# muonzoo/cutesdr

Hardware: AMD Instinct MI355X
Metric: complex IQ MSamples/s through CFastFIR+demod chain; achieved HBM GB/s vs peak (higher is better)
Workload: dtype f32; 1 GPU; C3: 256 channels/GPU x 2^19 IQ samples, 16384-pt CFastFIR overlap-save (8193 taps, hop 8192), shared -5..+5 kHz filter @62.5 kS/s; channels_per_gpu=256, samples_per_channel=524288, fft_size=16384, parallelism=channels sharded x1, no data-path collective

## Files before the change

cutesdr_amd/csrc/capi_fastfir.hip:

```cpp
#include "capi_common.hpp"
#include "capi_internal.hpp"
#include <algorithm>
#include "fastfir_kernels.h"
#include "fastfir_design_kernels.h"
#include "host_math.hpp"
#include "patch_queue.hpp"
#include <cmath>
#include <cstdlib>
#include <cstring>
#include <vector>

using namespace csdr;

static int log2_of(int n)
{
    int l = 0;
    while ((1 << l) < n) l++;
    return ((1 << l) == n) ? l : -1;
}

struct csdr_fastfir_batch {
    int device, channels, n, log2n;
    int cus;
    hipStream_t last_stream;
    bool per_channel;
    float *d_h;
    float *d_h2;
    float *d_hist;
    int hist_cur;
    int dbg_stage; float *dbg_out;
    int variant;
    float *d_tw1, *d_tw2;
    double flo, fhi, off, fs;
    std::vector<std::vector<cd>> resp;
    std::vector<int> perm, perm2;
    PatchQueue patches;
    std::vector<DesignJob> jobs;
    std::vector<int> job_of;
    std::vector<char> stale;
    double *d_win = nullptr, *d_tw = nullptr;
    int *d_perm = nullptr, *d_perm2 = nullptr;
    double *d_resp = nullptr;
    hipEvent_t ev_design = nullptr;
};

static void cancel_job(csdr_fastfir_batch *b, int slot)
{
    const int i = b->job_of[slot];
    if (i < 0) return;
    b->job_of[slot] = -1;
    if ((size_t)i + 1 != b->jobs.size()) { b->jobs[i] = b->jobs.back(); b->job_of[b->jobs[i].slot] = i; }
    b->jobs.pop_back();
}

static void queue_job(csdr_fastfir_batch *b, int slot, double nfc, double nfs)
{
    const DesignJob j{slot, 0, nfc, nfs};
    if (b->job_of[slot] >= 0) b->jobs[b->job_of[slot]] = j;
    else { b->job_of[slot] = (int)b->jobs.size(); b->jobs.push_back(j); }
    b->stale[slot] = 1;
}

static int flush_control(csdr_fastfir_batch *b, hipStream_t s)
{
    if (b->jobs.empty()) return b->patches.flush(s);
    unsigned char *h = nullptr, *d = nullptr;
    int rc = b->patches.take(b->jobs.size() * sizeof(DesignJob), &h, &d);
    if (rc) return rc;
    memcpy(h, b->jobs.data(), b->jobs.size() * sizeof(DesignJob));
    rc = b->patches.launch(s);
    hipError_t e = hipSuccess;
    if (!rc) {
        DesignArgs a;
        a.jobs = (const DesignJob *)d; a.win = b->d_win; a.tw = b->d_tw; a.perm = b->d_perm; a.perm2 = b->d_perm2;
        a.h = b->d_h; a.h2 = b->d_h2; a.resp = b->d_resp;
        e = fastfir_design_launch(b->log2n, a, (int)b->jobs.size(), s);
        if (e == hipSuccess) {
            for (const DesignJob &j : b->jobs) b->job_of[j.slot] = -1;
            b->jobs.clear();
            if (!b->ev_design) e = hipEventCreateWithFlags(&b->ev_design, hipEventDisableTiming);
            if (e == hipSuccess) e = hipEventRecord(b->ev_design, s);
        }
    }
    const int rr = b->patches.retire(s);
    if (rc) return rc;
    if (e != hipSuccess) return fail(CSDR_EHIP, "filter design launch: %s", hipGetErrorString(e));
    return rr;
}

static int fetch_mirror(csdr_fastfir_batch *b, int slot)
{
    if (!b->stale[slot]) return CSDR_OK;
    const int rc = flush_control(b, b->last_stream);
    if (rc) return rc;
    if (b->ev_design) CSDR_HIP(hipEventSynchronize(b->ev_design));
    CSDR_HIP(hipMemcpy(b->resp[slot].data(), b->d_resp + (size_t)slot * 2 * b->n, sizeof(cd) * (size_t)b->n, hipMemcpyDeviceToHost));
    b->stale[slot] = 0;
    return CSDR_OK;
}

static int design_state(csdr_fastfir_batch *b)
{
    if (b->d_resp) return CSDR_OK;
    const size_t n = (size_t)b->n, p = n / 2 + 1;
    const auto win = fastfir_window((int)p);
    const auto tw = design_twiddles(n);
    if (!b->d_win) CSDR_HIP(hipMalloc((void **)&b->d_win, p * sizeof(double)));
    if (!b->d_tw) CSDR_HIP(hipMalloc((void **)&b->d_tw, n * sizeof(double)));
    if (!b->d_perm) CSDR_HIP(hipMalloc((void **)&b->d_perm, n * sizeof(int)));
    if (!b->d_perm2) CSDR_HIP(hipMalloc((void **)&b->d_perm2, n * sizeof(int)));
    CSDR_HIP(hipMemcpy(b->d_win, win->data(), p * sizeof(double), hipMemcpyHostToDevice));
    CSDR_HIP(hipMemcpy(b->d_tw, tw.data(), n * sizeof(double), hipMemcpyHostToDevice));
    CSDR_HIP(hipMemcpy(b->d_perm, b->perm.data(), n * sizeof(int), hipMemcpyHostToDevice));
    CSDR_HIP(hipMemcpy(b->d_perm2, b->perm2.data(), n * sizeof(int), hipMemcpyHostToDevice));
    CSDR_HIP(hipMalloc((void **)&b->d_resp, (size_t)b->channels * n * sizeof(cd)));
    return CSDR_OK;
}

static void build_perm(csdr_fastfir_batch *b)
{
    const int T = b->n / 32;
    b->perm.resize(b->n);
    for (int j = 0; j < 16; j++)
        for (int t = 0; t < T; t++)
            for (int e = 0; e < 2; e++)
                b->perm[(j * T + t) * 2 + e] = fastfir_bin_of(b->log2n, t, 2 * j + e);
    b->perm2.clear();
    {
        b->perm2.resize(b->n);
        for (int j = 0; j < 16; j++)
            for (int t = 0; t < T; t++)
                for (int e = 0; e < 2; e++) b->perm2[(j * T + t) * 2 + e] = fastfir2_bin_of(b->log2n, t, j, e);
    }
}

static int upload_response(csdr_fastfir_batch *b, int slot, const std::vector<cd> &H)
{
    std::vector<float> dev(2 * (size_t)b->n);
    for (int pass = 0; pass < 2; pass++) {
        const std::vector<int> &perm = pass ? b->perm2 : b->perm;
        float *dst = pass ? b->d_h2 : b->d_h;
        if (perm.empty() || !dst) continue;
        for (int i = 0; i < b->n; i++) {
            const cd v = H[perm[i]];
            dev[2 * i] = (float)v.real();
            dev[2 * i + 1] = (float)v.imag();
        }
        const int rc = b->patches.add(dst + (size_t)slot * 2 * b->n, dev.data(), dev.size() * sizeof(float));
        if (rc) return rc;
    }
    return CSDR_OK;
}

static int set_response(csdr_fastfir_batch *b, int slot, const std::vector<cd> &H)
{
    cancel_job(b, slot);
    const int rc = upload_response(b, slot, H);
    if (rc) return rc;
    b->resp[slot] = H;
    b->stale[slot] = 0;
    return CSDR_OK;
}

extern "C" {

csdr_fastfir_batch *csdr_fastfir_batch_create(int device, int channels, int fft_size)
{
    const int l2 = log2_of(fft_size);
    if (l2 < 11 || l2 > 14 || channels < 1) {
        fail(CSDR_EINVAL, "fft_size must be 2048..16384 (power of two), channels >= 1");
        return nullptr;
    }
    if (!device_ok(device)) return nullptr;
    csdr_fastfir_batch *b = new csdr_fastfir_batch();
    b->device = device; b->channels = channels; b->n = fft_size; b->log2n = l2;
    b->per_channel = false; b->hist_cur = 0; b->dbg_stage = 0; b->dbg_out = nullptr;
    b->last_stream = nullptr;
    {
        int cus = 0;
        if (hipDeviceGetAttribute(&cus, hipDeviceAttributeMultiprocessorCount, device) != hipSuccess || cus <= 0) cus = 256;
        b->cus = cus;
    }
    {
        const char *v = getenv("CSDR_FASTFIR_VARIANT");
        b->variant = (v && atoi(v) == 0) ? 0 : 2;
    }
    b->d_h = b->d_h2 = b->d_hist = b->d_tw1 = b->d_tw2 = nullptr;
    b->flo = -1.0; b->fhi = 1.0; b->off = 1.0; b->fs = 1.0;
    build_perm(b);
    const size_t hbytes = (size_t)fft_size * 8, histbytes = 2 * (size_t)channels * (fft_size / 2) * 8;
    std::vector<float> tw1(2 * 1024), tw2(2 * 1024);
    for (int i = 0; i < 1024; i++) {
        const double a = kTwoPi * (double)i / (double)fft_size;
        tw1[2 * i] = (float)std::cos(a); tw1[2 * i + 1] = (float)std::sin(a);
    }
    for (int k = 0; k < 32; k++)
        for (int i = 0; i < 32; i++) {
            const double a = kTwoPi * (double)(i * k) / 1024.0;
            tw2[2 * (k * 32 + i)] = (float)std::cos(a); tw2[2 * (k * 32 + i) + 1] = (float)std::sin(a);
        }
    bool ok = hipMalloc((void **)&b->d_h, hbytes) == hipSuccess &&
              hipMalloc((void **)&b->d_h2, hbytes) == hipSuccess && hipMemset(b->d_h2, 0, hbytes) == hipSuccess &&
              hipMalloc((void **)&b->d_hist, histbytes) == hipSuccess &&
              hipMalloc((void **)&b->d_tw1, 8192) == hipSuccess &&
              hipMalloc((void **)&b->d_tw2, 8192) == hipSuccess &&
              hipMemset(b->d_h, 0, hbytes) == hipSuccess &&
              hipMemset(b->d_hist, 0, histbytes) == hipSuccess &&
              hipMemcpy(b->d_tw1, tw1.data(), 8192, hipMemcpyHostToDevice) == hipSuccess &&
              hipMemcpy(b->d_tw2, tw2.data(), 8192, hipMemcpyHostToDevice) == hipSuccess;
    if (!ok) {
        fail(CSDR_ENOMEM, "device allocation failed: %s", hipGetErrorString(hipGetLastError()));
        csdr_fastfir_batch_destroy(b);
        return nullptr;
    }
    b->resp.assign(1, std::vector<cd>(fft_size, cd(0, 0)));
    b->job_of.assign(channels, -1);
    b->stale.assign(channels, 0);
    return b;
}

void csdr_fastfir_batch_destroy(csdr_fastfir_batch *b)
{
    if (!b) return;
    (void)hipSetDevice(b->device);
    if (b->d_h) (void)hipFree(b->d_h);
    if (b->d_h2) (void)hipFree(b->d_h2);
    if (b->d_hist) (void)hipFree(b->d_hist);
    if (b->d_tw1) (void)hipFree(b->d_tw1);
    if (b->d_tw2) (void)hipFree(b->d_tw2);
    if (b->ev_design) { (void)hipEventSynchronize(b->ev_design); (void)hipEventDestroy(b->ev_design); }
    if (b->d_win) (void)hipFree(b->d_win);
    if (b->d_tw) (void)hipFree(b->d_tw);
    if (b->d_perm) (void)hipFree(b->d_perm);
    if (b->d_perm2) (void)hipFree(b->d_perm2);
    if (b->d_resp) (void)hipFree(b->d_resp);
    delete b;
}

int csdr_fastfir_batch_setup(csdr_fastfir_batch *b, int channel, double flo, double fhi,
                             double offset, double fs)
{
    if (!b || channel < -1 || channel >= b->channels) return fail(CSDR_EINVAL, "bad handle/channel");
    if (!device_ok(b->device)) return CSDR_EHIP;
    if (channel < 0) {
        if (!b->per_channel && flo == b->flo && fhi == b->fhi && offset == b->off && fs == b->fs) return 0;
        b->flo = flo; b->fhi = fhi; b->off = offset; b->fs = fs;
    }
    std::vector<cd> H;
    if (!fastfir_design(b->n, flo, fhi, offset, fs, H))
        return fail(CSDR_EINVAL, "filter parameter error (reference keeps the previous taps)");
    if (channel >= 0 && !b->per_channel) {
        { const int rcm = fetch_mirror(b, 0); if (rcm) return rcm; }
        { const int rcp = flush_control(b, b->last_stream); if (rcp) return rcp; }
        CSDR_HIP(hipDeviceSynchronize());
        float *nh = nullptr;
        const size_t one = (size_t)b->n * 8;
        CSDR_HIP(hipMalloc((void **)&nh, one * b->channels));
        for (int c = 0; c < b->channels; c++)
            CSDR_HIP(hipMemcpy((char *)nh + one * c, b->d_h, one, hipMemcpyDeviceToDevice));
        CSDR_HIP(hipFree(b->d_h));
        b->d_h = nh;
        if (b->d_h2) {
            float *nh2 = nullptr;
            CSDR_HIP(hipMalloc((void **)&nh2, one * b->channels));
            for (int c = 0; c < b->channels; c++)
                CSDR_HIP(hipMemcpy((char *)nh2 + one * c, b->d_h2, one, hipMemcpyDeviceToDevice));
            CSDR_HIP(hipFree(b->d_h2));
            b->d_h2 = nh2;
        }
        b->resp.resize(b->channels, b->resp[0]);
        b->per_channel = true;
    }
    if (channel < 0 && b->per_channel) {
        for (int c = 0; c < b->channels; c++) {
            int rc = set_response(b, c, H);
            if (rc) return rc;
        }
    } else {
        int rc = set_response(b, channel < 0 ? 0 : channel, H);
        if (rc) return rc;
    }
    return 1;
}

int csdr_fastfir_batch_setup_many(csdr_fastfir_batch *b, int n, const int *channel, const double *flo, const double *fhi,
                                  const double *offset, const double *fs, int *status)
{
    if (!have_device()) return CSDR_EHIP;
    if (!b || n < 0 || (n > 0 && (!channel || !flo || !fhi || !offset || !fs || !status)))
        return fail(CSDR_EINVAL, "bad handle, negative count or null array");
    for (int i = 0; i < n; i++)
        if (channel[i] < -1 || channel[i] >= b->channels) return fail(CSDR_EINVAL, "entry %d: channel %d", i, channel[i]);
    if (n == 0) return CSDR_OK;
    if (!device_ok(b->device)) return CSDR_EHIP;
    { const int rc = design_state(b); if (rc) return rc; }
    for (int i = 0; i < n; i++) {
        const int ch = channel[i];
        if (ch < 0) {
            if (!b->per_channel && flo[i] == b->flo && fhi[i] == b->fhi && offset[i] == b->off && fs[i] == b->fs) { status[i] = 0; continue; }
            b->flo = flo[i]; b->fhi = fhi[i]; b->off = offset[i]; b->fs = fs[i];
        }
        double nfc, nfs;
        if (!fastfir_design_job(flo[i], fhi[i], offset[i], fs[i], nfc, nfs)) { status[i] = CSDR_EINVAL; continue; }
        if (ch >= 0 && !b->per_channel) {
            const int rc = csdr_fastfir_batch_setup(b, ch, flo[i], fhi[i], offset[i], fs[i]);
            if (rc < 0) { for (int j = i; j < n; j++) status[j] = rc; return rc; }
        }
        if (ch < 0 && b->per_channel) for (int c = 0; c < b->channels; c++) queue_job(b, c, nfc, nfs);
        else queue_job(b, ch < 0 ? 0 : ch, nfc, nfs);
        status[i] = 1;
    }
    return CSDR_OK;
}

int csdr_fastfir_batch_reset(csdr_fastfir_batch *b)
{
    if (!b) return fail(CSDR_EINVAL, "bad handle");
    if (!device_ok(b->device)) return CSDR_EHIP;
    CSDR_HIP(hipMemset(b->d_hist, 0, 2 * (size_t)b->channels * (b->n / 2) * 8));
    return CSDR_OK;
}

int csdr_fastfir_batch_get_response(csdr_fastfir_batch *b, int channel, double *h_out)
{
    if (!b || !h_out || channel < 0 || channel >= b->channels) return fail(CSDR_EINVAL, "bad argument");
    const int slot = b->per_channel ? channel : 0;
    if (b->stale[slot]) {
        if (!device_ok(b->device)) return CSDR_EHIP;
        const int rc = fetch_mirror(b, slot);
        if (rc) return rc;
    }
    const std::vector<cd> &H = b->resp[slot];
    memcpy(h_out, H.data(), sizeof(cd) * H.size());
    return CSDR_OK;
}

int csdr_fastfir_batch_process(csdr_fastfir_batch *b, const float *d_in, long long in_stride,
                               int n_per_channel, float *d_out, long long out_stride,
                               void *stream, int blocks_per_wg)
{
    if (!b || !d_in || !d_out) return fail(CSDR_EINVAL, "bad handle or null buffer");
    const int L = b->n / 2;
    if (n_per_channel <= 0 || n_per_channel % L != 0)
        return fail(CSDR_EINVAL, "n_per_channel (%d) must be a positive multiple of the hop %d", n_per_channel, L);
    if (in_stride < n_per_channel || out_stride < n_per_channel)
        return fail(CSDR_EINVAL, "channel stride shorter than n_per_channel");
    if (((uintptr_t)d_in | (uintptr_t)d_out) & 15 || (in_stride & 1) || (out_stride & 1))
        return fail(CSDR_EINVAL, "buffers must be 16-byte aligned and strides even");
    if ((long long)n_per_channel * 8 >= (1ll << 31))
        return fail(CSDR_EINVAL, "n_per_channel (%d) too large for one call: at most %d samples", n_per_channel, (1 << 28) - L);
    if (!device_ok(b->device)) return CSDR_EHIP;
    hipStream_t s = (hipStream_t)stream;
    b->last_stream = s;
    { const int rcp = flush_control(b, s); if (rcp) return rcp; }
    FastFirArgs a;
    const size_t hist_half = (size_t)b->channels * L * 2;
    a.in = (const v2f_h *)d_in; a.out = (v2f_h *)d_out;
    a.hist = (const v2f_h *)(b->d_hist + b->hist_cur * hist_half);
    a.hist_next = (v2f_h *)(b->d_hist + (b->hist_cur ^ 1) * hist_half);
    a.h = (const v4f_h *)b->d_h; a.tw1 = (const v2f_h *)b->d_tw1; a.tw2 = (const v2f_h *)b->d_tw2;
    a.in_stride = in_stride; a.out_stride = out_stride;
    a.h_stride = b->per_channel ? b->n / 2 : 0;
    a.channels = b->channels;
    a.nblocks = n_per_channel / L;
    if (blocks_per_wg <= 0) {
        const long per_cu = b->n >= 16384 ? 1 : (b->n >= 8192 ? 2 : (b->n >= 4096 ? 4 : 8));
        const long slots = (long)b->cus * per_cu;
        long best_runs = 1; double best_eff = -1.0;
        const long max_runs = std::min<long>(a.nblocks, std::max<long>(1, 4 * ((slots + b->channels - 1) / b->channels)));
        for (long runs = 1; runs <= max_runs; runs++) {
            const long wgs = runs * b->channels;
            const double eff = (double)wgs / (double)(((wgs + slots - 1) / slots) * slots);
            if (eff > best_eff + 1e-9) { best_eff = eff; best_runs = runs; }
        }
        blocks_per_wg = (int)((a.nblocks + best_runs - 1) / best_runs);
    }
    if (blocks_per_wg > a.nblocks) blocks_per_wg = a.nblocks;
    a.blocks_per_run = blocks_per_wg;
    a.runs = (a.nblocks + blocks_per_wg - 1) / blocks_per_wg;
    a.dbg_stage = b->dbg_stage; a.dbg = (v2f_h *)b->dbg_out;
    if (b->variant >= 2) {
        a.h = (const v4f_h *)b->d_h2;
        CSDR_HIP(fastfir2_launch(b->log2n, a, s));
    }
    else CSDR_HIP(fastfir_launch(b->log2n, a, s));
    b->hist_cur ^= 1;
    return CSDR_OK;
}

int csdr__fastfir_batch_copy_row(csdr_fastfir_batch *dst, int dr, csdr_fastfir_batch *src, int sr)
{
    if (!dst || !src || dst->n != src->n || dr < 0 || dr >= dst->channels || sr < 0 || sr >= src->channels)
        return fail(CSDR_EINVAL, "bad argument");
    if (!device_ok(dst->device)) return CSDR_EHIP;
    CSDR_HIP(hipDeviceSynchronize());
    const int L = dst->n / 2;
    const size_t shalf = (size_t)src->channels * L * 2, dhalf = (size_t)dst->channels * L * 2;
    CSDR_HIP(hipMemcpy(dst->d_hist + dst->hist_cur * dhalf + (size_t)dr * L * 2,
                       src->d_hist + src->hist_cur * shalf + (size_t)sr * L * 2, (size_t)L * 8, hipMemcpyDeviceToDevice));
    const int sslot = src->per_channel ? sr : 0;
    { const int rcm = fetch_mirror(src, sslot); if (rcm) return rcm; }
    const std::vector<cd> &H = src->resp[sslot];
    if (dst->channels > 1 && !dst->per_channel) return fail(CSDR_ESTATE, "destination rows share one filter");
    const int slot = dst->per_channel ? dr : 0;
    int rc = set_response(dst, slot, H);
    if (rc) return rc;
    dst->flo = dst->fhi = dst->off = dst->fs = std::nan("");
    return CSDR_OK;
}

int csdr__fastfir_set_variant(csdr_fastfir_batch *b, int variant)
{
    if (!b || (variant != 0 && variant != 2)) return CSDR_EINVAL;
    b->variant = variant;
    return CSDR_OK;
}

int csdr__dbg_fastfir_stage(csdr_fastfir_batch *b, int stage, float *d_dbg)
{
    if (!b) return CSDR_EINVAL;
    b->dbg_stage = stage; b->dbg_out = d_dbg;
    return CSDR_OK;
}

}

struct csdr_fastfir {
    csdr_fastfir_batch *b;
    int n, pending;
    PinnedBuf pin_in, pin_out;
    hipStream_t s = nullptr;
    float *d_in, *d_out;
    size_t cap;
};

static int ensure_cap(csdr_fastfir *f, size_t samples)
{
    if (samples <= f->cap) return CSDR_OK;
    if (f->d_in) (void)hipFree(f->d_in);
    if (f->d_out) (void)hipFree(f->d_out);
    f->d_in = f->d_out = nullptr; f->cap = 0;
    CSDR_HIP(hipMalloc((void **)&f->d_in, samples * 8));
    CSDR_HIP(hipMalloc((void **)&f->d_out, samples * 8));
    f->cap = samples;
    return CSDR_OK;
}

extern "C" {

csdr_fastfir *csdr_fastfir_create(int device, int fft_size)
{
    csdr_fastfir_batch *b = csdr_fastfir_batch_create(device, 1, fft_size);
    if (!b) return nullptr;
    csdr_fastfir *f = new csdr_fastfir();
    f->b = b; f->n = fft_size; f->pending = 0; f->d_in = f->d_out = nullptr; f->cap = 0;
    if (hipStreamCreateWithFlags(&f->s, hipStreamNonBlocking) != hipSuccess) { csdr_fastfir_destroy(f); fail(CSDR_EHIP, "stream creation failed"); return nullptr; }
    return f;
}

void csdr_fastfir_destroy(csdr_fastfir *f)
{
    if (!f) return;
    (void)hipSetDevice(f->b->device);
    if (f->d_in) (void)hipFree(f->d_in);
    if (f->d_out) (void)hipFree(f->d_out);
    if (f->s) { (void)hipStreamSynchronize(f->s); (void)hipStreamDestroy(f->s); }
    csdr_fastfir_batch_destroy(f->b);
    delete f;
}

int csdr_fastfir_setup(csdr_fastfir *f, double flo, double fhi, double offset, double fs)
{
    if (!f) return fail(CSDR_EINVAL, "bad handle");
    return csdr_fastfir_batch_setup(f->b, -1, flo, fhi, offset, fs);
}

int csdr_fastfir_process(csdr_fastfir *f, int n, const double *in_iq, double *out_iq)
{
    if (!f || n < 0 || (n > 0 && (!in_iq || !out_iq))) return fail(CSDR_EINVAL, "bad argument");
    if (n == 0) return 0;
    if (!device_ok(f->b->device)) return CSDR_EHIP;
    const int L = f->n / 2;
    int rc = f->pin_in.reserve(2 * ((size_t)f->pending + n));
    if (rc) return rc;
    cvt_to_f32(f->pin_in.p + 2 * (size_t)f->pending, in_iq, 2 * (size_t)n);
    const int avail = f->pending + n;
    const int nproc = (avail / L) * L;
    if (nproc == 0) { f->pending = avail; return 0; }
    if ((rc = ensure_cap(f, (size_t)nproc))) { f->pending = avail; return rc; }
    if ((rc = f->pin_out.reserve(2 * (size_t)nproc))) { f->pending = avail; return rc; }
    CSDR_HIP(hipMemcpyAsync(f->d_in, f->pin_in.p, (size_t)nproc * 8, hipMemcpyHostToDevice, f->s));
    rc = csdr_fastfir_batch_process(f->b, f->d_in, nproc, nproc, f->d_out, nproc, (void *)f->s, 0);
    if (rc) {
        (void)hipStreamSynchronize(f->s);
        f->pending = avail;
        return rc;
    }
    CSDR_HIP(hipMemcpyAsync(f->pin_out.p, f->d_out, (size_t)nproc * 8, hipMemcpyDeviceToHost, f->s));
    CSDR_HIP(hipStreamSynchronize(f->s));
    cvt_to_f64(out_iq, f->pin_out.p, 2 * (size_t)nproc);
    f->pending = avail - nproc;
    if (f->pending > 0) memmove(f->pin_in.p, f->pin_in.p + 2 * (size_t)nproc, 2 * (size_t)f->pending * sizeof(float));
    return nproc;
}

}
```

cutesdr_amd/csrc/capi_hosttest.hip:

```cpp
#include "capi_common.hpp"
#include "host_math.hpp"
#include "dc_host.hpp"
#include "pc_host.hpp"
#include "display_plan.hpp"
#include "testgen_host.hpp"
#include "scope_host.hpp"
#include "fastfir_kernels.h"
#include <cstring>

using namespace csdr;

extern "C" {

int csdr__host_fastfir_design(int n, double flo, double fhi, double off, double fs, double *h_out)
{
    std::vector<cd> H;
    if (!fastfir_design(n, flo, fhi, off, fs, H)) return -1;
    memcpy(h_out, H.data(), sizeof(cd) * n);
    return 0;
}
int csdr__host_design_job(double flo, double fhi, double off, double fs, double *nfc, double *nfs)
{
    return fastfir_design_job(flo, fhi, off, fs, *nfc, *nfs) ? 0 : -1;
}
int csdr__host_fastfir_bin_of(int log2n, int t, int r) { return fastfir_bin_of(log2n, t, r); }

int csdr__host_dc_plan(double in_rate, double bw, int *codes, double *out_rate, int *warmup)
{
    DcPlan p = dc_make_plan(in_rate, bw);
    for (int i = 0; i < p.nstages; i++) codes[i] = p.kind[i];
    *out_rate = p.out_rate; *warmup = p.W;
    return p.nstages;
}
int csdr__host_dc_stage_taps(double in_rate, double bw, int s, double *h)
{
    DcPlan p = dc_make_plan(in_rate, bw);
    if (s < 0 || s >= p.nstages) return -1;
    const DcStage &st = p.st[s];
    const int L = st.hist + (p.kind[s] == 3 ? 2 : 1);
    for (int i = 0; i < L; i++) h[i] = 0;
    if (st.center >= 0) h[st.center] = st.ccoef;
    for (int q = 0; q < st.npairs; q++) { h[st.a[q]] = st.c[q]; h[st.b[q]] = st.c[q]; }
    return L;
}
void csdr__host_dc_nco(double freq, double cw, double in_rate, unsigned long long *inc, double *stored)
{
    DcHostChan c;
    c.in_rate = in_rate; c.cw_offset = cw;
    c.set_frequency(freq);
    *inc = c.inc; *stored = c.nco_freq;
}
int csdr__host_fir_design(int kind, double scale, double astop, double fpass, double fstop, double fs,
                          double hilbert_off, double *coef, double *icoef, double *qcoef)
{
    HostFir f;
    if (kind == 0) f.init_lp(scale, astop, fpass, fstop, fs);
    else f.init_hp(scale, astop, fpass, fstop, fs);
    if (hilbert_off != 0.0) f.gen_hilbert(hilbert_off);
    for (int i = 0; i < f.ntaps; i++) { coef[i] = f.coef[i]; icoef[i] = f.icoef[i]; qcoef[i] = f.qcoef[i]; }
    return f.ntaps;
}
void csdr__host_iir_design(int kind, double f0, double q, double fs, double *c5)
{
    PcIir f;
    iir_design(f, kind, f0, q, fs);
    c5[0] = f.b0; c5[1] = f.b1; c5[2] = f.b2; c5[3] = f.a1; c5[4] = f.a2;
}
void csdr__host_agc_params(int on, int hang, int thresh, int manual, int slope, int decay, double fs, double *out12)
{
    HostAgc h;
    PcAgc d;
    memset(&d, 0, sizeof(d));
    h.set(d, on != 0, hang != 0, thresh, manual, slope, decay, fs);
    out12[0] = d.knee; out12[1] = d.gain_slope; out12[2] = d.fixed_gain; out12[3] = d.manual_gain;
    out12[4] = d.att_rise; out12[5] = d.att_fall; out12[6] = d.dec_rise; out12[7] = d.dec_fall;
    out12[8] = d.dly_n; out12[9] = d.win_n; out12[10] = d.hang_time; out12[11] = 0;
}

void csdr__host_display_plan(const int *state5, long long n, int N, long long *out8)
{
    DisplayState s;
    s.pos = state5[0]; s.skip = state5[1]; s.counter = state5[2]; s.gated = state5[3]; s.ready = state5[4];
    const DisplayPlan p = display_plan(s, n, N);
    out8[0] = p.start; out8[1] = p.step; out8[2] = p.count;
    out8[3] = p.next.pos; out8[4] = p.next.skip; out8[5] = p.next.counter; out8[6] = p.next.gated; out8[7] = p.next.ready;
}
int csdr__host_display_skip_value(double sample_rate, int fft_size, int max_display_rate)
{
    return display_skip_value(sample_rate, fft_size, max_display_rate);
}

unsigned long long csdr__host_tg_first_crossing(double x0, double d, double limit, int strict, double *value)
{
    return tg::first_crossing(x0, d, limit, strict != 0, value);
}
double csdr__host_tg_value_at(double x0, double d, unsigned long long index) { return tg::value_at(x0, d, index); }
void csdr__host_tg_pulse_pattern(double fs, double period, double width, unsigned long long *K, unsigned long long *W)
{
    tg::Gen g;
    g.fs = fs; g.period = period; g.width = width;
    g.pulse_pattern();
    *K = g.K; *W = g.W;
}
void *csdr__host_tg_create(void) { tg::Gen *g = new tg::Gen(); g->reset(); g->on = true; return g; }
void csdr__host_tg_destroy(void *h) { delete (tg::Gen *)h; }
void csdr__host_tg_slot(void *h, int what, double v)
{
    tg::Gen &g = *(tg::Gen *)h;
    switch (what) {
    case 0: g.on_sweep_start(v); break;
    case 1: g.on_sweep_stop(v); break;
    case 2: g.on_sweep_rate(v); break;
    case 3: g.on_pulse_width(v); break;
    case 4: g.on_pulse_period(v); break;
    case 5: g.on_signal_pwr(v); break;
    case 6: g.on_noise_pwr(v); break;
    default: g.reset(); break;
    }
}
int csdr__host_tg_run(void *h, int n, double fs, unsigned long long *phase, int *gate)
{
    tg::Gen &g = *(tg::Gen *)h;
    if (g.fs != fs) { g.fs = fs; g.pulse_valid = false; g.reset(); }
    tg::ChanParam p;
    g.pulse((uint32_t)n, p);
    uint32_t done = 0;
    int launches = 0;
    while (done < (uint32_t)n) {
        p.nseg = 0;
        const uint32_t lo = done;
        done += g.advance(done, (uint32_t)n - done, p);
        launches++;
        for (uint32_t j = lo; j < done; j++) {
            uint32_t s = 0;
            for (uint32_t k = 1; k < p.nseg; k++) s += p.seg_start[k] <= j;
            const uint64_t t = j - p.seg_start[s];
            const tg::u128 P = (((tg::u128)p.seg_p[s][1] << 64) | p.seg_p[s][0])
                + (((tg::u128)p.seg_d[s][1] << 64) | p.seg_d[s][0]) * (tg::u128)t
                + (((tg::u128)p.seg_d2[s][1] << 64) | p.seg_d2[s][0]) * (tg::u128)(t * (t - 1) / 2);
            phase[j] = (uint64_t)(P >> 64);
            const uint64_t m = (uint64_t)j + 1;
            const uint64_t pos = m < p.wrap1 ? p.pos0 + m : (m - p.wrap1) % p.period;
            gate[j] = !p.gate_on || pos < p.width;
        }
    }
    return launches;
}

long long csdr__host_scope_emissions(long long inpos, int pos, double pix, double sr, int w, long long n, long long max_out,
                                     long long *samples, long long *end3)
{
    const sc::Plan p = sc::make_plan(inpos, pos, pix, sr, w, n);
    for (long long e = 0; e < p.emits && e < max_out; e++) samples[e] = p.sample(e);
    end3[0] = p.emits; end3[1] = p.pos_end; end3[2] = p.inpos_end;
    return p.emits;
}
void csdr__host_scope_settings(int span_ms, int display_rate, double sr, int w, double *pix, int *skip)
{
    *pix = sc::pixel_time(span_ms, w); *skip = sc::skip_value(span_ms, display_rate, sr);
}
void csdr__host_scope_free_run(long long cnt, int skip, long long m, long long *out3)
{
    const sc::FreeRun r = sc::free_run(cnt, skip, m);
    out3[0] = r.displays; out3[1] = r.last; out3[2] = r.cnt;
}
struct HostScope {
    sc::Chan ch;
    sc::ChanState st;
    int w = 100, h = 100;
    int ring[2 * sc::kMaxW], screen[2 * sc::kMaxW];
};
void *csdr__host_scope_create(void)
{
    HostScope *s = new HostScope();
    memset(&s->st, 0, sizeof(s->st)); s->st.skipcounter = -2;
    memset(s->ring, 0, sizeof(s->ring)); memset(s->screen, 0, sizeof(s->screen));
    s->ch.derive(s->w);
    return s;
}
void csdr__host_scope_destroy(void *h) { delete (HostScope *)h; }
void csdr__host_scope_slot(void *h, int what, int v, int v2)
{
    HostScope &s = *(HostScope *)h;
    switch (what) {
    case 0: s.w = v; s.h = v2; s.ch.reset(v); break;
    case 1: s.ch.on_horz_span(v, s.w); break;
    case 2: s.ch.on_display_rate(v); break;
    case 3: s.ch.on_trigger_mode(v, s.w); break;
    case 4: s.ch.level = v; break;
    case 5: s.ch.vert = v; break;
    case 6: s.ch.reset(s.w); break;
    default: s.ch.time_plot_done(); break;
    }
}
long long csdr__host_scope_put(void *h, const float *re, const float *im, int n, double fs)
{
    HostScope &s = *(HostScope *)h;
    sc::ChanParam par;
    s.ch.prepare(n, fs, s.w, par);
    sc::ChanState &st = s.st;
    int *ring = s.ring, *screen = s.screen;
    const int w = s.w;
    if (par.flags & sc::F_RESET) memset(ring, 0, sizeof(s.ring));
    sc::apply_flags(st, par.flags);
    if (par.n > 0) {
        const sc::Plan pl = sc::make_plan(st.inpos, st.pos, par.pix, par.sr, w, par.n);
        const long long E = pl.emits;
        const int pos0 = st.pos;
        auto get = [&](long long e, int &a, int &b) { const long long k = pl.sample(e); a = sc::sat_int(re[k]); b = im ? sc::sat_int(im[k]) : 0; };
        long long trig = -1;
        if (sc::searches(st, par))
            for (long long e = 0; e < E && trig < 0; e++) {
                int cur, prv, t;
                get(e, cur, t);
                if (e == 0) prv = st.prev; else get(e - 1, prv, t);
                if (sc::crossing(par.mode, par.level, cur, prv)) trig = e;
            }
        const sc::Display d = sc::decide(st, par, w, E, trig);
        if (d.at >= 0)
            for (int i = 0; i < w; i++) {
                int a, b, slot = 0;
                const long long e = sc::screen_source(d, i, w, pos0, &slot);
                if (e >= 0) get(e, a, b); else { a = ring[slot]; b = ring[sc::kMaxW + slot]; }
                screen[i] = a; screen[sc::kMaxW + i] = b;
            }
        for (long long e = E > w ? E - w : 0; e < E; e++) {
            int a, b;
            get(e, a, b);
            const int slot = (int)((pos0 + e) % w);
            ring[slot] = a; ring[sc::kMaxW + slot] = b;
        }
        int t;
        if (E > 0) get(E - 1, st.prev, t);
        st.inpos = pl.inpos_end; st.pos = pl.pos_end;
    }
    return st.emits;
}
void csdr__host_scope_get(void *h, long long *state7, int *screen_re, int *screen_im)
{
    HostScope &s = *(HostScope *)h;
    const sc::ChanState &st = s.st;
    state7[0] = st.inpos; state7[1] = st.pos; state7[2] = st.prev; state7[3] = st.trigstate; state7[4] = st.trigcounter;
    state7[5] = st.trigbufpos; state7[6] = st.skipcounter;
    memcpy(screen_re, s.screen, sizeof(int) * s.w); memcpy(screen_im, s.screen + sc::kMaxW, sizeof(int) * s.w);
}
int csdr__host_scope_sat_int(double x) { return sc::sat_int(x); }

}
```

cutesdr_amd/csrc/fastfir2_kernels.hip:

```cpp
#define CSDR_FMA_BFLY 1
#define CSDR_PLAIN_CONST_FMA 1
#include "launch_once.hpp"
#include "fastfir_dev.hpp"
#include "fastfir_kernels.h"

namespace csdr {

#define CSDR_SB() __builtin_amdgcn_sched_barrier(0)

#ifndef K1_LDAUX
#define K1_LDAUX 2
#endif
#ifndef K1_STAUX
#define K1_STAUX 2
#endif
#ifndef K1_HREG
#define K1_HREG 8
#endif
#ifndef K1_HREG4K
#define K1_HREG4K 4
#endif
#ifndef K1_W1_FETCH_MAX_R0
#define K1_W1_FETCH_MAX_R0 2
#endif
#ifndef K1_HREG2K
#define K1_HREG2K 8
#endif

#ifdef CSDR_K1_STAMPS
#define CSDR_STAMP(i)                                                                         \
    do {                                                                                      \
        CSDR_SB();                                                                            \
        unsigned long long now_;                                                              \
        asm volatile("s_memtime %0\n\ts_waitcnt lgkmcnt(0)" : "=s"(now_)::"memory");         \
        CSDR_SB();                                                                            \
        acc_[i] += now_ - last_;                                                              \
        last_ = now_;                                                                         \
    } while (0)
#else
#define CSDR_STAMP(i) do { } while (0)
#endif

#define CSDR_PRIO(p) __builtin_amdgcn_s_setprio(p)

#ifdef K1_ABLATE
__device__ __forceinline__ void keep_alive(v4f v) { asm volatile("" ::"v"(v)); }
#endif

template <int LOG2N>
struct K1Cfg {
    using Base = FastFirCfg<LOG2N>;
    static constexpr int VW = LOG2N == 12 ? 2 : (LOG2N == 11 ? 4 : 1);
    static constexpr int TV = Base::T;
    static constexpr int T = VW * TV;
    static constexpr int LDS_BYTES = (VW * Base::LDS_DATA + 1024) * 8;
};

template <int LOG2N>
__global__ __launch_bounds__(K1Cfg<LOG2N>::T) __attribute__((amdgpu_waves_per_eu(2, 2)))
void fastfir_os2_kernel(FastFirArgs a)
{
    CSDR_WG_TRACE_SCOPE(a.trace, WGT_FF);
    using Cfg = FastFirCfg<LOG2N>;
    constexpr int N = Cfg::N, T = Cfg::T, R0 = Cfg::R0, G = Cfg::G, L = N / 2;
    constexpr int HALF = R0 / 2;
    constexpr int VW = K1Cfg<LOG2N>::VW;
    constexpr int HREG = LOG2N == 12 ? K1_HREG4K : (LOG2N == 11 ? K1_HREG2K : K1_HREG);
    static_assert(R0 == 16 || R0 == 8 || R0 == 4 || R0 == 2, "the grouped outer pass is written for N = 2048 ... 16384");
    auto block_barrier = [] {
        if constexpr (LOG2N == 11) {
            __builtin_amdgcn_fence(__ATOMIC_RELEASE, "wavefront"); __builtin_amdgcn_wave_barrier(); __builtin_amdgcn_fence(__ATOMIC_ACQUIRE, "wavefront");
        } else {
            __syncthreads();
        }
    };
    extern __shared__ __attribute__((aligned(16))) unsigned char smem_raw[];
    const int t = VW == 1 ? (int)threadIdx.x : (int)threadIdx.x % T, vw = VW == 1 ? 0 : (int)threadIdx.x / T;
    v2f *lds = reinterpret_cast<v2f *>(smem_raw) + vw * Cfg::LDS_DATA;
    v2f *tw2 = reinterpret_cast<v2f *>(smem_raw) + VW * Cfg::LDS_DATA;
    if constexpr (VW > 1) {
        for (int i = threadIdx.x; i < 1024; i += VW * T) tw2[i] = a.tw2[i];
        __syncthreads();
    }

    int wg = blockIdx.x * VW + vw, ch, run;
    if ((a.channels & 7) == 0) {
        int xcd = wg & 7, slot = wg >> 3;
        ch = (slot / a.runs) * 8 + xcd;
        run = slot % a.runs;
    } else {
        ch = wg / a.runs;
        run = wg % a.runs;
    }
    const int b0 = run * a.blocks_per_run;
    int b1 = b0 + a.blocks_per_run;
    if (b1 > a.nblocks) b1 = a.nblocks;
#if defined(__HIP_DEVICE_COMPILE__) && !defined(__gfx950__)
#error "fastfir_os2_kernel<12> relies on gfx950's s_barrier ignoring terminated waves (two virtual workgroups per workgroup)"
#endif
    if (ch >= a.channels || b0 >= b1) return;

    if constexpr (VW == 1)
        for (int i = t; i < 1024; i += T) tw2[i] = a.tw2[i];

    const rsrc_t r_in = make_rsrc(a.in + (long)ch * a.in_stride, (unsigned)a.nblocks * L * 8u);
    const rsrc_t r_hist = make_rsrc(a.hist + (long)ch * L, L * 8u);
    const rsrc_t r_out = make_rsrc(a.out + (long)ch * a.out_stride, (unsigned)a.nblocks * L * 8u);
    const rsrc_t r_h = make_rsrc(a.h + (long)ch * a.h_stride, N * 8u);
    constexpr int PSTEP = 2 * T, PSTEP_LDS = PSTEP + 2 * (PSTEP / 32), PSTEP_B = PSTEP * 8;
    const int voff = t * 16;
    auto load_half = [&](rsrc_t r, int soff, v2f (&dst)[16]) {
#pragma unroll
        for (int n1 = 0; n1 < HALF; n1++)
#pragma unroll
            for (int pp = 0; pp < G / 2; pp++) {
                v4f v = buf_load16_aux<K1_LDAUX>(r, voff + pp * PSTEP_B, soff + n1 * 8192);
                dst[(2 * pp) * HALF + n1] = v2f{v.x, v.y};
                dst[(2 * pp + 1) * HALF + n1] = v2f{v.z, v.w};
            }
    };

    constexpr bool W1_RESIDENT = R0 > K1_W1_FETCH_MAX_R0;
    auto w_pair = [&](int pp) { return *reinterpret_cast<const v4f *>(a.tw1 + PSTEP * pp + 2 * t); };
    v2f w1[R0 > 2 ? G : 1];
    auto load_w1 = [&] {
        if constexpr (R0 > 2) {
#pragma unroll
            for (int pp = 0; pp < G / 2; pp++) { const v4f v = w_pair(pp); w1[2 * pp] = v2f{v.x, v.y}; w1[2 * pp + 1] = v2f{v.z, v.w}; }
        }
    };
    load_w1();
    v2f pw[G][R0];
    if constexpr (R0 > 2) {
#pragma unroll
        for (int e = 0; e < G; e++) twiddle_powers<R0>(opaque(w1[e]), pw[e]);
    }

    v4f hv[16];
#pragma unroll
    for (int j = 0; j < HREG; j++) hv[j] = buf_load16(r_h, t * 16, j * (T * 16));
#ifdef K1_ABLATE
    v4f habl = {1.0f, 0.0f, 1.0f, 0.0f};
    asm volatile("" : "+v"(habl));
    v2f twabl = {0.8f, 0.6f};
    asm volatile("" : "+v"(twabl));
#endif
    v2f x[32];
    v2f hp[16], hq[16];

    if (b0 == 0) load_half(r_hist, 0, hp);
    else load_half(r_in, (b0 - 1) * (L * 8), hp);
    load_half(r_in, b0 * (L * 8), hq);

    const int sb = t >> 5, sn = t & 31;
    v2f *const col = lds + lds_pad(1024 * sb) + sn;
    const v2f *const twc = tw2 + sn;
    v2f *const rowp = lds + 34 * t;
    v2f *const outer = lds + lds_pad(2 * t);
    constexpr int OUTER_ROW = 1024 + 2 * (1024 / 32);

#ifdef K1_CYC
    const unsigned long long cyc0_ = __builtin_amdgcn_s_memtime(), rt0_ = __builtin_amdgcn_s_memrealtime();
#endif
#ifdef CSDR_K1_STAMPS
    unsigned long long acc_[16] = {0, 0, 0, 0, 0, 0, 0, 0, 0, 0, 0, 0, 0, 0, 0, 0}, last_;
    asm volatile("s_memtime %0\n\ts_waitcnt lgkmcnt(0)" : "=s"(last_)::"memory");
#endif
    auto one_block = [&](const int b, v2f (&oldh)[16], v2f (&newh)[16]) {
        CSDR_SB();
        CSDR_PRIO(1);
        {
            v2f y[G][R0];
            static_for<0, HALF>([&](auto N1) {
                static_for<0, G>([&](auto E) {
                    constexpr int e = E.value, n1 = N1.value, po = bitrev<R0>(n1), pn = bitrev<R0>(HALF + n1);
                    y[e][po] = oldh[e * HALF + n1]; y[e][pn] = newh[e * HALF + n1];
                });
            });
            if constexpr (R0 == 2) {
                static_for<0, G>([&](auto E) { bfly_dit<0, +1>(y[E.value][0], y[E.value][1]); });
            } else {
                static_for<0, (R0 >= 8 ? R0 / 4 : 1)>([&](auto Gg) {
                    static_for<0, G>([&](auto E) { dit_head4<Gg.value, R0, +1>(y[E.value]); });
                });
            }
            CSDR_SB();
            load_half(r_in, (b + 1 < a.nblocks ? b + 1 : a.nblocks - 1) * (L * 8), oldh);
            CSDR_SB();
            CSDR_PRIO(0);
            v4f wv[16];
            if constexpr (R0 == 16) {
                static_for<0, R0 / 4 + 1>([&](auto Ii) {
                    constexpr int i = Ii.value;
                    if constexpr (i < R0 / 4) {
                        dit_tail<i, R0, +1>(y[0]);
                        dit_tail<i, R0, +1>(y[1]);
                        static_for<0, 4>([&](auto P) {
                            constexpr int k0 = i + 4 * P.value;
                            if constexpr (k0 != 0) {
                                y[0][k0] = cmul(y[0][k0], pw[0][k0]);
                                y[1][k0] = cmul(y[1][k0], pw[1][k0]);
                            }
                            wv[k0] = store_operand(y[0][k0], y[1][k0]);
                        });
                    }
                    if constexpr (i > 0) {
                        CSDR_STORE_GROUP_BEGIN();
                        static_for<0, 4>([&](auto P) {
                            constexpr int k0 = (i - 1) + 4 * P.value;
                            *reinterpret_cast<v4f *>(outer + OUTER_ROW * k0) = wv[k0];
                        });
                        CSDR_STORE_GROUP_END();
                    } else {
                        CSDR_SB();
                    }
                });
            } else if constexpr (R0 == 2) {
                v4f wq[8];
                static_for<0, 8>([&](auto PP) { wq[PP.value] = w_pair(PP.value); });
                static_for<0, 5>([&](auto Ii) {
                    constexpr int i = Ii.value;
                    if constexpr (i < 4) {
                        static_for<0, 2>([&](auto Q) {
                            constexpr int pp = 2 * i + Q.value;
                            y[2 * pp][1] = cmul(y[2 * pp][1], v2f{wq[pp].x, wq[pp].y});
                            y[2 * pp + 1][1] = cmul(y[2 * pp + 1][1], v2f{wq[pp].z, wq[pp].w});
                            wv[pp] = store_operand(y[2 * pp][0], y[2 * pp + 1][0]);
                            wv[8 + pp] = store_operand(y[2 * pp][1], y[2 * pp + 1][1]);
                        });
                    }
                    if constexpr (i > 0) {
                        CSDR_STORE_GROUP_BEGIN();
                        static_for<0, 2>([&](auto Q) {
                            constexpr int pp = 2 * (i - 1) + Q.value;
                            *reinterpret_cast<v4f *>(outer + PSTEP_LDS * pp) = wv[pp];
                            *reinterpret_cast<v4f *>(outer + OUTER_ROW + PSTEP_LDS * pp) = wv[8 + pp];
                        });
                        CSDR_STORE_GROUP_END();
                    } else {
                        CSDR_SB();
                    }
                });
            } else {
                constexpr int NG = 4, RPG = R0 / NG;
                static_for<0, NG + 1>([&](auto Ii) {
                    constexpr int i = Ii.value;
                    if constexpr (i < NG) {
                        if constexpr (R0 == 8)
                            static_for<0, G>([&](auto E) { bfly_dit<4 * i, +1>(y[E.value][i], y[E.value][i + 4]); });
                        static_for<0, RPG>([&](auto P) {
                            constexpr int k0 = i + NG * P.value;
                            static_for<0, G>([&](auto E) {
                                if constexpr (k0 != 0) y[E.value][k0] = cmul(y[E.value][k0], pw[E.value][k0]);
                            });
                            static_for<0, G / 2>([&](auto PP) {
                                wv[k0 * (G / 2) + PP.value] = store_operand(y[2 * PP.value][k0], y[2 * PP.value + 1][k0]);
                            });
                        });
                    }
                    if constexpr (i > 0) {
                        CSDR_STORE_GROUP_BEGIN();
                        static_for<0, RPG>([&](auto P) {
                            constexpr int k0 = (i - 1) + NG * P.value;
                            static_for<0, G / 2>([&](auto PP) {
                                *reinterpret_cast<v4f *>(outer + OUTER_ROW * k0 + PSTEP_LDS * PP.value) = wv[k0 * (G / 2) + PP.value];
                            });
                        });
                        CSDR_STORE_GROUP_END();
                    } else {
                        CSDR_SB();
                    }
                });
            }
        }
        CSDR_STAMP(0);
#ifdef ABL_BAR
        __builtin_amdgcn_fence(__ATOMIC_RELEASE, "wavefront"); __builtin_amdgcn_wave_barrier(); __builtin_amdgcn_fence(__ATOMIC_ACQUIRE, "wavefront");
#else
        block_barrier();
#endif
        CSDR_STAMP(1);

        CSDR_PRIO(3);
        {
            auto fetch = [&](auto Gg) {
                static_for<0, 4>([&](auto Q) {
                    constexpr int p = 4 * Gg.value + Q.value;
                    x[p] = lds_ld8(col + 34 * bitrev<32>(p));
                });
            };
            static_for<0, 3>(fetch);
            CSDR_SB();
            static_for<0, 8>([&](auto Gg) {
                if constexpr (Gg.value + 3 < 8) fetch(std::integral_constant<int, Gg.value + 3>{});
                dit_head4<Gg.value, 32, +1>(x);
                if constexpr ((Gg.value & 1) == 1) CSDR_SB();
            });
            CSDR_STAMP(7);
            dit_single<8, 32, +1>(x);
            CSDR_SB();
            v2f tw[2][4];
#ifdef ABL_TW
            static_for<1, 4>([&](auto P) { tw[0][P.value] = twabl; });
#else
            static_for<1, 4>([&](auto P) { tw[0][P.value] = lds_ld8(twc + 32 * (8 * P.value)); });
#endif
            CSDR_SB();
            CSDR_STAMP(8);
            static_for<0, 9>([&](auto Ii) {
                constexpr int i = Ii.value;
                if constexpr (i < 7)
#ifdef ABL_TW
                    static_for<0, 4>([&](auto P) { tw[(i + 1) & 1][P.value] = twabl; });
#else
                    static_for<0, 4>([&](auto P) { tw[(i + 1) & 1][P.value] = lds_ld8(twc + 32 * (i + 1 + 8 * P.value)); });
#endif
                if constexpr (i < 8) {
#ifdef ABL_H
                    hv[2 * i] = habl; hv[2 * i + 1] = habl;
#else
                    if constexpr (2 * i >= HREG) hv[2 * i] = buf_load16(r_h, t * 16, (2 * i) * (T * 16));
                    if constexpr (2 * i + 1 >= HREG) hv[2 * i + 1] = buf_load16(r_h, t * 16, (2 * i + 1) * (T * 16));
#endif
                    dit_tail<i, 32, +1>(x);
                    static_for<0, 4>([&](auto P) {
                        constexpr int k1 = i + 8 * P.value;
                        if constexpr (k1 != 0) x[k1] = cmul(x[k1], tw[i & 1][P.value]);
                    });
                }
                if constexpr (i > 0)
                    static_for<0, 4>([&](auto P) {
                        constexpr int k1 = (i - 1) + 8 * P.value;
                        lds_st8(col + 34 * k1, x[k1]);
                    });
                CSDR_SB();
            });
        }
        CSDR_STAMP(2);
        __builtin_amdgcn_fence(__ATOMIC_RELEASE, "wavefront");
        __builtin_amdgcn_wave_barrier();
        __builtin_amdgcn_fence(__ATOMIC_ACQUIRE, "wavefront");

        CSDR_PRIO(2);
        {
            v2f y[32];
            static_for<0, 4>([&](auto Q) {
                static_for<0, 4>([&](auto P) {
                    constexpr int j = Q.value + 4 * P.value;
                    const v4f v = *reinterpret_cast<const v4f *>(rowp + 2 * j);
                    x[bitrev<32>(2 * j)] = v2f{v.x, v.y};
                    x[bitrev<32>(2 * j + 1)] = v2f{v.z, v.w};
                });
            });
            CSDR_SB();
            static_for<0, 4>([&](auto Q) {
                dit_head4<bitrev<8>(2 * Q.value), 32, +1>(x);
                dit_head4<bitrev<8>(2 * Q.value + 1), 32, +1>(x);
                CSDR_SB();
            });
            dit_single<8, 32, +1>(x);
            CSDR_SB();
            static_for<0, 8>([&](auto Ii) {
                constexpr int i = Ii.value, g = bitrev<8>(i);
                dit_tail<i, 32, +1>(x);
                y[4 * g] = x[i]; y[4 * g + 1] = x[i + 16]; y[4 * g + 2] = x[i + 8]; y[4 * g + 3] = x[i + 24];
                dit_head4_tw<g, 32, -1>(y, v2f{hv[2 * i].x, hv[2 * i].y}, v2f{hv[2 * i].z, hv[2 * i].w},
                                        v2f{hv[2 * i + 1].x, hv[2 * i + 1].y}, v2f{hv[2 * i + 1].z, hv[2 * i + 1].w});
                if constexpr ((i & 1) == 1) CSDR_SB();
            });
#pragma unroll
            for (int i = 0; i < 32; i++) x[i] = y[i];
            CSDR_PRIO(1);
            dit_single<8, 32, -1>(x);
            CSDR_SB();
            v4f wv[16];
            static_for<0, 5>([&](auto Q) {
                constexpr int q = Q.value;
                if constexpr (q < 4) {
                    dit_tail<2 * q, 32, -1>(x);
                    dit_tail<2 * q + 1, 32, -1>(x);
                    static_for<0, 4>([&](auto P) {
                        constexpr int j = q + 4 * P.value;
                        wv[j] = store_operand(x[2 * j], x[2 * j + 1]);
                    });
                }
                if constexpr (q > 0) {
                    CSDR_STORE_GROUP_BEGIN();
                    static_for<0, 4>([&](auto P) {
                        constexpr int j = (q - 1) + 4 * P.value;
                        *reinterpret_cast<v4f *>(rowp + 2 * j) = wv[j];
                    });
                    CSDR_STORE_GROUP_END();
                } else {
                    CSDR_SB();
                }
            });
        }
        CSDR_STAMP(3);
        __builtin_amdgcn_fence(__ATOMIC_RELEASE, "wavefront");
        __builtin_amdgcn_wave_barrier();
        __builtin_amdgcn_fence(__ATOMIC_ACQUIRE, "wavefront");

        CSDR_PRIO(0);
        {
            v2f tw[32];
            auto fetch = [&](auto Gg) {
                static_for<0, 4>([&](auto Q) {
                    constexpr int r = 4 * Gg.value + Q.value;
                    x[r] = lds_ld8(col + 34 * bitrev<32>(r));
                });
                static_for<0, 4>([&](auto Q) {
                    constexpr int r = 4 * Gg.value + Q.value;
#ifdef ABL_TW
                    if constexpr (r != 0) tw[r] = twabl;
#else
                    if constexpr (r != 0) tw[r] = lds_ld8(twc + 32 * bitrev<32>(r));
#endif
                });
            };
            static_for<0, 2>(fetch);
            CSDR_SB();
            static_for<0, 8>([&](auto Gg) {
                constexpr int g = Gg.value;
                if constexpr (g + 2 < 8) fetch(std::integral_constant<int, g + 2>{});
                dit_head4_conjtw<g, 32, -1, g == 0>(x, tw[4 * g], tw[4 * g + 1], tw[4 * g + 2], tw[4 * g + 3]);
                if constexpr ((g & 1) == 1) CSDR_SB();
            });
            dit_single<8, 32, -1>(x);
            CSDR_SB();
            static_for<0, 9>([&](auto I) {
                constexpr int i = I.value;
                if constexpr (i < 8) dit_tail<i, 32, -1>(x);
                if constexpr (i > 0)
                    static_for<0, 4>([&](auto P) {
                        constexpr int n1 = (i - 1) + 8 * P.value;
                        lds_st8(col + 34 * n1, x[n1]);
                    });
                CSDR_SB();
            });
        }
        CSDR_STAMP(4);
#ifdef ABL_BAR
        __builtin_amdgcn_fence(__ATOMIC_RELEASE, "wavefront"); __builtin_amdgcn_wave_barrier(); __builtin_amdgcn_fence(__ATOMIC_ACQUIRE, "wavefront");
#else
        block_barrier();
#endif
        CSDR_STAMP(5);

        CSDR_PRIO(3);
        {
            v2f y[G][R0];
            static_for<0, R0>([&](auto Rr) {
                constexpr int r = Rr.value, k0 = bitrev<R0>(r);
                static_for<0, G / 2>([&](auto PP) {
                    const v4f v = *reinterpret_cast<const v4f *>(outer + OUTER_ROW * k0 + PSTEP_LDS * PP.value);
                    y[2 * PP.value][r] = v2f{v.x, v.y};
                    y[2 * PP.value + 1][r] = v2f{v.z, v.w};
                });
            });
            if constexpr (R0 > 2) {
                if constexpr (!W1_RESIDENT) load_w1();
#pragma unroll
                for (int e = 0; e < G; e++) twiddle_powers<R0>(opaque(w1[e]), pw[e]);
                CSDR_SB();
                static_for<0, (R0 >= 8 ? R0 / 4 : 1)>([&](auto Gg) {
                    constexpr int g = Gg.value;
                    static_for<0, G>([&](auto E) {
                        constexpr int e = E.value;
                        dit_head4_conjtw<g, R0, -1, g == 0>(y[e], pw[e][bitrev<R0>(4 * g)], pw[e][bitrev<R0>(4 * g + 1)],
                                                            pw[e][bitrev<R0>(4 * g + 2)], pw[e][bitrev<R0>(4 * g + 3)]);
                    });
                    if constexpr ((g & 1) == 1) CSDR_SB();
                });
            }
            CSDR_PRIO(2);
            v4f sv[8];
            if constexpr (R0 == 16) {
                static_for<0, R0 / 4 + 1>([&](auto I) {
                    constexpr int i = I.value;
                    if constexpr (i < R0 / 4) {
                        dit_tail_upper<i, R0, -1>(y[0]);
                        dit_tail_upper<i, R0, -1>(y[1]);
                        sv[2 * i] = store_operand(y[0][i + 8], y[1][i + 8]);
                        sv[2 * i + 1] = store_operand(y[0][i + 12], y[1][i + 12]);
                    }
                    if constexpr (i > 0) {
                        CSDR_STORE_GROUP_BEGIN();
#ifdef ABL_GST
                        keep_alive(sv[2 * (i - 1)]); keep_alive(sv[2 * (i - 1) + 1]);
#else
                        buf_store16_aux<K1_STAUX>(r_out, voff, b * (L * 8) + (i - 1) * 8192, sv[2 * (i - 1)]);
                        buf_store16_aux<K1_STAUX>(r_out, voff, b * (L * 8) + (i - 1 + 4) * 8192, sv[2 * (i - 1) + 1]);
#endif
                        CSDR_STORE_GROUP_END();
                    } else {
                        CSDR_SB();
                    }
                });
            } else if constexpr (R0 == 2) {
                v4f wq[8];
                static_for<0, 8>([&](auto PP) { wq[PP.value] = w_pair(PP.value); });
                static_for<0, 5>([&](auto I) {
                    constexpr int i = I.value;
                    if constexpr (i < 4) {
                        static_for<0, 2>([&](auto Q) {
                            constexpr int pp = 2 * i + Q.value;
                            const v2f d0 = y[2 * pp][0] - cmul_conj(y[2 * pp][1], v2f{wq[pp].x, wq[pp].y});
                            const v2f d1 = y[2 * pp + 1][0] - cmul_conj(y[2 * pp + 1][1], v2f{wq[pp].z, wq[pp].w});
                            sv[pp] = store_operand(d0, d1);
                        });
                    }
                    if constexpr (i > 0) {
                        CSDR_STORE_GROUP_BEGIN();
                        static_for<0, 2>([&](auto Q) {
                            constexpr int pp = 2 * (i - 1) + Q.value;
                            buf_store16_aux<K1_STAUX>(r_out, voff + pp * PSTEP_B, b * (L * 8), sv[pp]);
                        });
                        CSDR_STORE_GROUP_END();
                    } else {
                        CSDR_SB();
                    }
                });
            } else {
                constexpr int NG = HALF;
                static_for<0, NG + 1>([&](auto I) {
                    constexpr int i = I.value;
                    if constexpr (i < NG) {
                        if constexpr (R0 == 8)
                            static_for<0, G>([&](auto E) { bfly_dit_lower<4 * i, -1>(y[E.value][i], y[E.value][i + 4]); });
                        static_for<0, G / 2>([&](auto PP) {
                            sv[i * (G / 2) + PP.value] = store_operand(y[2 * PP.value][HALF + i], y[2 * PP.value + 1][HALF + i]);
                        });
                    }
                    if constexpr (i > 0) {
                        CSDR_STORE_GROUP_BEGIN();
                        static_for<0, G / 2>([&](auto PP) {
                            buf_store16_aux<K1_STAUX>(r_out, voff + PP.value * PSTEP_B, b * (L * 8) + (i - 1) * 8192,
                                                      sv[(i - 1) * (G / 2) + PP.value]);
                        });
                        CSDR_STORE_GROUP_END();
                    } else {
                        CSDR_SB();
                    }
                });
            }
        }
        CSDR_STAMP(6);
    };
    __builtin_amdgcn_s_waitcnt(0x0f70);
    int b = b0;
    for (; b + 1 < b1; b += 2) {
        one_block(b, hp, hq);
        one_block(b + 1, hq, hp);
    }
    const bool odd_tail = b < b1;
    if (odd_tail) one_block(b, hp, hq);

#ifdef K1_CYC
    if (a.dbg && t == 0) {
        unsigned long long *o = reinterpret_cast<unsigned long long *>(a.dbg) + (long)blockIdx.x * 2;
        o[0] = __builtin_amdgcn_s_memtime() - cyc0_;
        o[1] = __builtin_amdgcn_s_memrealtime() - rt0_;
    }
#endif
#ifdef CSDR_K1_STAMPS
    if (a.dbg && (t & 63) == 0) {
        unsigned long long *o = reinterpret_cast<unsigned long long *>(a.dbg) + ((long)blockIdx.x * (T / 64) + (t >> 6)) * 16;
        for (int i = 0; i < 16; i++) o[i] = acc_[i];
    }
#endif
    if (b1 == a.nblocks) {
        const rsrc_t r_hn = make_rsrc(a.hist_next + (long)ch * L, L * 8u);
        v4f sv[8];
#pragma unroll
        for (int n1 = 0; n1 < HALF; n1++)
#pragma unroll
            for (int pp = 0; pp < G / 2; pp++)
                sv[n1 * (G / 2) + pp] = odd_tail ? store_operand(hq[(2 * pp) * HALF + n1], hq[(2 * pp + 1) * HALF + n1])
                                                 : store_operand(hp[(2 * pp) * HALF + n1], hp[(2 * pp + 1) * HALF + n1]);
        CSDR_STORE_GROUP_BEGIN();
#pragma unroll
        for (int n1 = 0; n1 < HALF; n1++)
#pragma unroll
            for (int pp = 0; pp < G / 2; pp++) buf_store16(r_hn, voff + pp * PSTEP_B, n1 * 8192, sv[n1 * (G / 2) + pp]);
        CSDR_STORE_GROUP_END();
    }
}

template <int LOG2N>
static hipError_t launch2_one(const FastFirArgs &a, hipStream_t stream)
{
    using Cfg = K1Cfg<LOG2N>;
    hipError_t e = CSDR_MAX_LDS_ONCE(&fastfir_os2_kernel<LOG2N>, Cfg::LDS_BYTES);
    if (e != hipSuccess) return e;
#ifdef CSDR_WG_TRACE
    FastFirArgs b = a;
    b.trace = wgtrace_next();
    hipLaunchKernelGGL((fastfir_os2_kernel<LOG2N>), dim3((a.channels * a.runs + Cfg::VW - 1) / Cfg::VW), dim3(Cfg::T),
                       Cfg::LDS_BYTES, stream, b);
    return hipGetLastError();
#endif
    hipLaunchKernelGGL((fastfir_os2_kernel<LOG2N>), dim3((a.channels * a.runs + Cfg::VW - 1) / Cfg::VW), dim3(Cfg::T),
                       Cfg::LDS_BYTES, stream, a);
    return hipGetLastError();
}

hipError_t fastfir2_launch(int log2n, const FastFirArgs &a, hipStream_t stream)
{
    switch (log2n) {
    case 11: return launch2_one<11>(a, stream);
    case 12: return launch2_one<12>(a, stream);
    case 13: return launch2_one<13>(a, stream);
    case 14: return launch2_one<14>(a, stream);
    default: return hipErrorInvalidValue;
    }
}

int fastfir2_bin_of(int log2n, int t, int j, int e)
{
    const int R0 = (1 << log2n) / 1024;
    const int i = j >> 1, h = j & 1;
    const int k2 = i + 8 * h + 16 * e;
    return (t >> 5) + R0 * ((t & 31) + 32 * k2);
}

}
```

cutesdr_amd/csrc/fastfir_design_kernels.h:

```cpp
#pragma once
#include <hip/hip_runtime.h>

namespace csdr {

struct DesignJob {
    int slot;
    int pad;
    double nfc, nfs;
};

struct DesignArgs {
    const DesignJob *jobs;
    const double *win;
    const double *tw;
    const int *perm, *perm2;
    float *h, *h2;
    double *resp;
};

hipError_t fastfir_design_launch(int log2n, const DesignArgs &a, int njobs, hipStream_t stream);

}
```

cutesdr_amd/csrc/fastfir_design_kernels.hip:

```cpp
#include "fastfir_design_kernels.h"
#include "launch_once.hpp"

namespace csdr {

namespace {

typedef double v2d __attribute__((ext_vector_type(2)));
typedef float v2f_d __attribute__((ext_vector_type(2)));

constexpr double kPiD = 3.14159265358979323846;
constexpr double kTwoPiD = 2.0 * kPiD;

template <int LOG2N>
struct DesignCfg {
    static constexpr int N = 1 << LOG2N;
    static constexpr bool IN_LDS = LOG2N <= 13;
    static constexpr int T = N / 8 > 1024 ? 1024 : N / 8;
    static constexpr int LDS_BYTES = IN_LDS ? N * 16 : 0;
};

template <int LOG2N>
__global__ __launch_bounds__(DesignCfg<LOG2N>::T) void fastfir_design_kernel(DesignArgs a)
{
#pragma clang fp contract(off)
    using Cfg = DesignCfg<LOG2N>;
    constexpr int N = Cfg::N, T = Cfg::T, P = N / 2 + 1, CENTRE = N / 4;
    extern __shared__ __attribute__((aligned(16))) unsigned char design_smem[];
    const DesignJob job = a.jobs[blockIdx.x];
    const int tid = threadIdx.x;
    v2d *row = reinterpret_cast<v2d *>(a.resp) + (size_t)job.slot * N;
    v2d *w;
    if constexpr (Cfg::IN_LDS) w = reinterpret_cast<v2d *>(design_smem);
    else w = row;

    for (int i = tid; i < N; i += T) {
        v2d v = {0.0, 0.0};
        if (i < P) {
            const double x = (double)(i - CENTRE);
            double z;
            if (i == CENTRE) z = 2.0 * job.nfc;
            else z = sin(kTwoPiD * x * job.nfc) / (kPiD * x) * a.win[i];
            v.x = z * cos(job.nfs * x) / (double)N;
            v.y = z * sin(job.nfs * x) / (double)N;
        }
        w[__brev((unsigned)i) >> (32 - LOG2N)] = v;
    }
    __syncthreads();

#pragma unroll 1
    for (int s = 1; s <= LOG2N; s++) {
        const int half = 1 << (s - 1);
        for (int q = tid; q < N / 2; q += T) {
            const int k = q & (half - 1);
            const int b = ((q - k) << 1) + k;
            const int j = k << (LOG2N - s);
            const double wr = a.tw[2 * j], wi = a.tw[2 * j + 1];
            const v2d u = w[b], x = w[b + half];
            v2d v;
            v.x = x.x * wr - x.y * wi;
            v.y = x.x * wi + x.y * wr;
            w[b] = u + v;
            w[b + half] = u - v;
        }
        __syncthreads();
    }

    v2f_d *h = reinterpret_cast<v2f_d *>(a.h) + (size_t)job.slot * N;
    v2f_d *h2 = reinterpret_cast<v2f_d *>(a.h2) + (size_t)job.slot * N;
    for (int i = tid; i < N; i += T) {
        const v2d p = w[a.perm[i]], p2 = w[a.perm2[i]];
        v2f_d f = {(float)p.x, (float)p.y}, f2 = {(float)p2.x, (float)p2.y};
        h[i] = f;
        h2[i] = f2;
        if constexpr (Cfg::IN_LDS) row[i] = w[i];
    }
}

template <int LOG2N>
hipError_t launch_one(const DesignArgs &a, int njobs, hipStream_t stream)
{
    using Cfg = DesignCfg<LOG2N>;
    if (Cfg::LDS_BYTES > 0) {
        hipError_t e = CSDR_MAX_LDS_ONCE((&fastfir_design_kernel<LOG2N>), Cfg::LDS_BYTES);
        if (e != hipSuccess) return e;
    }
    hipLaunchKernelGGL((fastfir_design_kernel<LOG2N>), dim3(njobs), dim3(Cfg::T), Cfg::LDS_BYTES, stream, a);
    return hipGetLastError();
}

}

hipError_t fastfir_design_launch(int log2n, const DesignArgs &a, int njobs, hipStream_t stream)
{
    if (njobs <= 0) return hipSuccess;
    switch (log2n) {
    case 11: return launch_one<11>(a, njobs, stream);
    case 12: return launch_one<12>(a, njobs, stream);
    case 13: return launch_one<13>(a, njobs, stream);
    case 14: return launch_one<14>(a, njobs, stream);
    default: return hipErrorInvalidValue;
    }
}

}
```

cutesdr_amd/csrc/fastfir_kernels.h:

```cpp
#pragma once
#include <hip/hip_runtime.h>
#include "wg_trace.hpp"

namespace csdr {

typedef float v2f_h __attribute__((ext_vector_type(2)));
typedef float v4f_h __attribute__((ext_vector_type(4)));

struct FastFirArgs {
    const v2f_h *in;
    const v2f_h *hist;
    v2f_h *hist_next;
    v2f_h *out;
    const v4f_h *h;
    const v2f_h *tw1;
    const v2f_h *tw2;
    long in_stride;
    long out_stride;
    long h_stride;
    int channels;
    int nblocks;
    int blocks_per_run;
    int runs;
    int dbg_stage;
    v2f_h *dbg;
#ifdef CSDR_WG_TRACE
    WgTraceArg trace;
#endif
};

hipError_t fastfir_launch(int log2n, const FastFirArgs &a, hipStream_t stream);
int fastfir_bin_of(int log2n, int t, int r);

hipError_t fastfir2_launch(int log2n, const FastFirArgs &a, hipStream_t stream);
int fastfir2_bin_of(int log2n, int t, int j, int e);

}
```

cutesdr_amd/csrc/fft_core.hpp:

```cpp
#pragma once
#include <hip/hip_runtime.h>

namespace csdr {

typedef float v2f __attribute__((ext_vector_type(2)));
typedef float v4f __attribute__((ext_vector_type(4)));

static constexpr float kCos32[32] = {
    1.0f, 0.98078528040323044913f, 0.92387953251128675613f, 0.83146961230254523708f,
    0.70710678118654752440f, 0.55557023301960222474f, 0.38268343236508977173f, 0.19509032201612826785f,
    0.0f, -0.19509032201612826785f, -0.38268343236508977173f, -0.55557023301960222474f,
    -0.70710678118654752440f, -0.83146961230254523708f, -0.92387953251128675613f, -0.98078528040323044913f,
    -1.0f, -0.98078528040323044913f, -0.92387953251128675613f, -0.83146961230254523708f,
    -0.70710678118654752440f, -0.55557023301960222474f, -0.38268343236508977173f, -0.19509032201612826785f,
    0.0f, 0.19509032201612826785f, 0.38268343236508977173f, 0.55557023301960222474f,
    0.70710678118654752440f, 0.83146961230254523708f, 0.92387953251128675613f, 0.98078528040323044913f};

#if defined(__HIP_DEVICE_COMPILE__) && !defined(CSDR_NO_PK_ASM)
#define CSDR_PK_ASM 1
#else
#define CSDR_PK_ASM 0
#endif

__host__ __device__ __forceinline__ v2f cmul_c(v2f a, v2f w)
{
    v2f wr = {-w.y, w.x};
    return a.xx * w + a.yy * wr;
}

__host__ __device__ __forceinline__ v2f cmul(v2f a, v2f w)
{
#if CSDR_PK_ASM
    v2f t, r;
    asm("v_pk_mul_f32 %0, %1, %2 op_sel:[0,0] op_sel_hi:[0,1]" : "=v"(t) : "v"(a), "v"(w));
    asm("v_pk_fma_f32 %0, %1, %2, %3 op_sel:[1,1,0] op_sel_hi:[1,0,1] neg_lo:[0,1,0]"
        : "=v"(r) : "v"(a), "v"(w), "v"(t));
    return r;
#else
    return cmul_c(a, w);
#endif
}
__host__ __device__ __forceinline__ v2f cmul_conj(v2f a, v2f w)
{
#if CSDR_PK_ASM
    v2f t, r;
    asm("v_pk_mul_f32 %0, %1, %2 op_sel:[0,0] op_sel_hi:[0,1] neg_hi:[0,1]" : "=v"(t) : "v"(a), "v"(w));
    asm("v_pk_fma_f32 %0, %1, %2, %3 op_sel:[1,1,0] op_sel_hi:[1,0,1]"
        : "=v"(r) : "v"(a), "v"(w), "v"(t));
    return r;
#else
    v2f wc = {w.x, -w.y}, wr = {w.y, w.x};
    return a.xx * wc + a.yy * wr;
#endif
}
template <int S>
__host__ __device__ __forceinline__ v2f add_jv(v2f u, v2f v)
{
#if CSDR_PK_ASM
    v2f r;
    if constexpr (S > 0)
        asm("v_pk_add_f32 %0, %1, %2 op_sel:[0,1] op_sel_hi:[1,0] neg_lo:[0,1]" : "=v"(r) : "v"(u), "v"(v));
    else
        asm("v_pk_add_f32 %0, %1, %2 op_sel:[0,1] op_sel_hi:[1,0] neg_hi:[0,1]" : "=v"(r) : "v"(u), "v"(v));
    return r;
#else
    return S > 0 ? v2f{u.x - v.y, u.y + v.x} : v2f{u.x + v.y, u.y - v.x};
#endif
}
template <int S>
__host__ __device__ __forceinline__ v2f sub_j(v2f u, v2f v)
{
#if CSDR_PK_ASM
    v2f r;
    if constexpr (S > 0)
        asm("v_pk_add_f32 %0, %1, %2 op_sel:[1,1] op_sel_hi:[0,0] neg_lo:[1,0] neg_hi:[0,1]" : "=v"(r) : "v"(u), "v"(v));
    else
        asm("v_pk_add_f32 %0, %1, %2 op_sel:[1,1] op_sel_hi:[0,0] neg_lo:[0,1] neg_hi:[1,0]" : "=v"(r) : "v"(u), "v"(v));
    return r;
#else
    return S > 0 ? v2f{-(u.y - v.y), u.x - v.x} : v2f{u.y - v.y, -(u.x - v.x)};
#endif
}

constexpr float kSqrtHalf = 0.70710678118654752440f;

template <int K, int SIGN>
__host__ __device__ __forceinline__ void bfly_dif(v2f &xa, v2f &xb)
{
    const v2f u = xa, v = xb;
    xa = u + v;
    if constexpr (K == 0) {
        xb = u - v;
    } else if constexpr (K == 8) {
        xb = sub_j<SIGN>(u, v);
    } else if constexpr (K == 4) {
        const v2f d = u - v;
        xb = add_jv<SIGN>(d, d) * kSqrtHalf;
    } else if constexpr (K == 12) {
        const v2f d = u - v;
        xb = add_jv<-SIGN>(d, d) * (-kSqrtHalf);
    } else {
        constexpr float c = kCos32[K];
        constexpr float s = (SIGN > 0 ? 1.0f : -1.0f) * kCos32[(K + 24) & 31];
        xb = cmul_c(u - v, v2f{c, s});
    }
}
#if CSDR_PK_ASM && defined(CSDR_FMA_BFLY)
#define CSDR_FMA_DIT 1
#else
#define CSDR_FMA_DIT 0
#endif
__host__ __device__ __forceinline__ void bfly_fma(v2f &xa, v2f &xb, v2f w)
{
#if CSDR_FMA_DIT
    v2f t, a;
    asm("v_pk_fma_f32 %0, %1, %2, %3 op_sel:[0,0,0] op_sel_hi:[0,1,1]" : "=v"(t) : "v"(xb), "v"(w), "v"(xa));
    asm("v_pk_fma_f32 %0, %1, %2, %3 op_sel:[1,1,0] op_sel_hi:[1,0,1] neg_lo:[0,1,0]" : "=v"(a) : "v"(xb), "v"(w), "v"(t));
    xb = xa * 2.0f - a;
    xa = a;
#else
    const v2f v = cmul(xb, w);
    const v2f u = xa;
    xa = u + v; xb = u - v;
#endif
}
__host__ __device__ __forceinline__ void bfly_fma_conj(v2f &xa, v2f &xb, v2f w)
{
#if CSDR_FMA_DIT
    v2f t, a;
    asm("v_pk_fma_f32 %0, %1, %2, %3 op_sel:[0,0,0] op_sel_hi:[0,1,1] neg_hi:[0,1,0]" : "=v"(t) : "v"(xb), "v"(w), "v"(xa));
    asm("v_pk_fma_f32 %0, %1, %2, %3 op_sel:[1,1,0] op_sel_hi:[1,0,1]" : "=v"(a) : "v"(xb), "v"(w), "v"(t));
    xb = xa * 2.0f - a;
    xa = a;
#else
    const v2f v = cmul_conj(xb, w);
    const v2f u = xa;
    xa = u + v; xb = u - v;
#endif
}

template <int K, int SIGN>
__host__ __device__ __forceinline__ void bfly_dit(v2f &xa, v2f &xb)
{
    const v2f u = xa;
#if CSDR_FMA_DIT
    if constexpr (K != 0 && K != 8) {
        constexpr float c = kCos32[K];
        constexpr float s = (SIGN > 0 ? 1.0f : -1.0f) * kCos32[(K + 24) & 31];
#ifdef CSDR_PLAIN_CONST_FMA
        const v2f w1 = {c, s}, w2 = {-s, c};
        const v2f t = __builtin_elementwise_fma(xb.xx, w1, u);
        const v2f a = __builtin_elementwise_fma(xb.yy, w2, t);
        xb = u * 2.0f - a;
        xa = a;
        return;
#else
        v2f t, a;
        const v2f w = {c, s};
        asm("v_pk_fma_f32 %0, %1, %2, %3 op_sel:[0,0,0] op_sel_hi:[0,1,1]" : "=v"(t) : "v"(xb), "s"(w), "v"(u));
        asm("v_pk_fma_f32 %0, %1, %2, %3 op_sel:[1,1,0] op_sel_hi:[1,0,1] neg_lo:[0,1,0]" : "=v"(a) : "v"(xb), "s"(w), "v"(t));
        xb = u * 2.0f - a;
        xa = a;
        return;
#endif
    }
#endif
    if constexpr (K == 0) {
        const v2f v = xb;
        xa = u + v; xb = u - v;
    } else if constexpr (K == 8) {
        const v2f v = xb;
        xa = add_jv<SIGN>(u, v); xb = add_jv<-SIGN>(u, v);
    } else if constexpr (K == 4) {
        const v2f v = add_jv<SIGN>(xb, xb) * kSqrtHalf;
        xa = u + v; xb = u - v;
    } else if constexpr (K == 12) {
        const v2f v = add_jv<-SIGN>(xb, xb) * (-kSqrtHalf);
        xa = u + v; xb = u - v;
    } else {
        constexpr float c = kCos32[K];
        constexpr float s = (SIGN > 0 ? 1.0f : -1.0f) * kCos32[(K + 24) & 31];
        const v2f v = cmul_c(xb, v2f{c, s});
        xa = u + v; xb = u - v;
    }
}

template <int R> __host__ __device__ constexpr int bitrev(int v)
{
    int r = 0;
    for (int m = 1; m < R; m <<= 1) { r = (r << 1) | (v & 1); v >>= 1; }
    return r;
}

template <int I, int N, class F>
__host__ __device__ __forceinline__ void static_for(F &&f)
{
    if constexpr (I < N) {
        f(std::integral_constant<int, I>{});
        static_for<I + 1, N>(f);
    }
}

template <int LEN, int R, int SIGN>
__host__ __device__ __forceinline__ void dif_stage(v2f (&x)[R])
{
    constexpr int H = LEN / 2;
    static_for<0, R / LEN>([&](auto B) {
        static_for<0, H>([&](auto I) {
            constexpr int a = B.value * LEN + I.value, b = a + H;
            bfly_dif<I.value *(32 / LEN), SIGN>(x[a], x[b]);
        });
    });
    if constexpr (LEN > 2) dif_stage<LEN / 2, R, SIGN>(x);
}
template <int R, int SIGN>
__host__ __device__ __forceinline__ void dft_dif(v2f (&x)[R])
{
    if constexpr (R > 1) dif_stage<R, R, SIGN>(x);
}

template <int LEN, int R, int SIGN>
__host__ __device__ __forceinline__ void dit_stage(v2f (&x)[R])
{
    constexpr int H = LEN / 2;
    static_for<0, R / LEN>([&](auto B) {
        static_for<0, H>([&](auto I) {
            constexpr int a = B.value * LEN + I.value, b = a + H;
            bfly_dit<I.value *(32 / LEN), SIGN>(x[a], x[b]);
        });
    });
    if constexpr (LEN < R) dit_stage<LEN * 2, R, SIGN>(x);
}
template <int R, int SIGN>
__host__ __device__ __forceinline__ void dft_dit(v2f (&x)[R])
{
    if constexpr (R > 1) dit_stage<2, R, SIGN>(x);
}

template <int LEN, int R, int SIGN>
__host__ __device__ __forceinline__ void dif_single(v2f (&x)[R])
{
    constexpr int H = LEN / 2;
    static_for<0, R / LEN>([&](auto B) {
        static_for<0, H>([&](auto I) {
            constexpr int a = B.value * LEN + I.value, b = a + H;
            bfly_dif<I.value *(32 / LEN), SIGN>(x[a], x[b]);
        });
    });
}
template <int LEN, int R, int SIGN>
__host__ __device__ __forceinline__ void dit_single(v2f (&x)[R])
{
    constexpr int H = LEN / 2;
    static_for<0, R / LEN>([&](auto B) {
        static_for<0, H>([&](auto I) {
            constexpr int a = B.value * LEN + I.value, b = a + H;
            bfly_dit<I.value *(32 / LEN), SIGN>(x[a], x[b]);
        });
    });
}
template <int I, int R, int SIGN>
__host__ __device__ __forceinline__ void dif_head(v2f (&x)[R])
{
    static_assert(R >= 8 && I < R / 4, "dif_head");
    constexpr int Q = R / 4;
    bfly_dif<I *(32 / R), SIGN>(x[I], x[I + 2 * Q]);
    bfly_dif<(I + Q) * (32 / R), SIGN>(x[I + Q], x[I + 3 * Q]);
    bfly_dif<I *(64 / R), SIGN>(x[I], x[I + Q]);
    bfly_dif<I *(64 / R), SIGN>(x[I + 2 * Q], x[I + 3 * Q]);
}
template <int G, int R, int SIGN>
__host__ __device__ __forceinline__ void dif_tail4(v2f (&x)[R])
{
    constexpr int a = 4 * G;
    bfly_dif<0, SIGN>(x[a], x[a + 2]);
    bfly_dif<8, SIGN>(x[a + 1], x[a + 3]);
    bfly_dif<0, SIGN>(x[a], x[a + 1]);
    bfly_dif<0, SIGN>(x[a + 2], x[a + 3]);
}
template <int G, int R, int SIGN>
__host__ __device__ __forceinline__ void dit_head4(v2f (&x)[R])
{
    constexpr int a = 4 * G;
    bfly_dit<0, SIGN>(x[a], x[a + 1]);
    bfly_dit<0, SIGN>(x[a + 2], x[a + 3]);
    bfly_dit<0, SIGN>(x[a], x[a + 2]);
    bfly_dit<8, SIGN>(x[a + 1], x[a + 3]);
}
template <int G, int R, int SIGN, bool FIRST_PLAIN>
__host__ __device__ __forceinline__ void dit_head4_conjtw(v2f (&x)[R], v2f t0, v2f t1, v2f t2, v2f t3)
{
    constexpr int a = 4 * G;
    if constexpr (!FIRST_PLAIN) x[a] = cmul_conj(x[a], t0);
    x[a + 2] = cmul_conj(x[a + 2], t2);
    bfly_fma_conj(x[a], x[a + 1], t1);
    bfly_fma_conj(x[a + 2], x[a + 3], t3);
    bfly_dit<0, SIGN>(x[a], x[a + 2]);
    bfly_dit<8, SIGN>(x[a + 1], x[a + 3]);
}
template <int G, int R, int SIGN>
__host__ __device__ __forceinline__ void dit_head4_tw(v2f (&x)[R], v2f t0, v2f t1, v2f t2, v2f t3)
{
    constexpr int a = 4 * G;
    x[a] = cmul(x[a], t0);
    x[a + 2] = cmul(x[a + 2], t2);
    bfly_fma(x[a], x[a + 1], t1);
    bfly_fma(x[a + 2], x[a + 3], t3);
    bfly_dit<0, SIGN>(x[a], x[a + 2]);
    bfly_dit<8, SIGN>(x[a + 1], x[a + 3]);
}
template <int K, int SIGN>
__host__ __device__ __forceinline__ void bfly_dit_lower(const v2f xa, v2f &xb)
{
    if constexpr (K == 0) {
        xb = xa - xb;
    } else if constexpr (K == 8) {
        xb = add_jv<-SIGN>(xa, xb);
    } else {
        constexpr float c = kCos32[K];
        constexpr float s = (SIGN > 0 ? 1.0f : -1.0f) * kCos32[(K + 24) & 31];
        const v2f w1 = {-c, -s}, w2 = {s, -c};
        const v2f t = __builtin_elementwise_fma(xb.xx, w1, xa);
        xb = __builtin_elementwise_fma(xb.yy, w2, t);
    }
}
template <int I, int R, int SIGN>
__host__ __device__ __forceinline__ void dit_tail_upper(v2f (&x)[R])
{
    static_assert(R >= 8 && I < R / 4, "dit_tail_upper");
    constexpr int Q = R / 4;
    bfly_dit<I *(64 / R), SIGN>(x[I], x[I + Q]);
    bfly_dit<I *(64 / R), SIGN>(x[I + 2 * Q], x[I + 3 * Q]);
    bfly_dit_lower<I *(32 / R), SIGN>(x[I], x[I + 2 * Q]);
    bfly_dit_lower<(I + Q) * (32 / R), SIGN>(x[I + Q], x[I + 3 * Q]);
}
template <int I, int R, int SIGN>
__host__ __device__ __forceinline__ void dit_tail(v2f (&x)[R])
{
    static_assert(R >= 8 && I < R / 4, "dit_tail");
    constexpr int Q = R / 4;
    bfly_dit<I *(64 / R), SIGN>(x[I], x[I + Q]);
    bfly_dit<I *(64 / R), SIGN>(x[I + 2 * Q], x[I + 3 * Q]);
    bfly_dit<I *(32 / R), SIGN>(x[I], x[I + 2 * Q]);
    bfly_dit<(I + Q) * (32 / R), SIGN>(x[I + Q], x[I + 3 * Q]);
}

template <int R>
__host__ __device__ __forceinline__ void twiddle_powers(v2f w, v2f (&pw)[R])
{
    pw[0] = v2f{1.0f, 0.0f};
    if constexpr (R > 1) pw[1] = w;
    static_for<2, R>([&](auto K) {
        constexpr int k = K.value;
        constexpr int hb = (k & (k - 1)) == 0 ? k / 2 : (1 << (31 - __builtin_clz(k)));
        pw[k] = cmul(pw[hb], pw[k - hb]);
    });
}

__host__ __device__ __forceinline__ v2f opaque(v2f v)
{
    asm volatile("" : "+v"(v));
    return v;
}

__device__ __forceinline__ v2f lds_ld8(const v2f *p)
{
    return __builtin_bit_cast(v2f, __hip_atomic_load(reinterpret_cast<const unsigned long long *>(p), __ATOMIC_RELAXED,
                                                     __HIP_MEMORY_SCOPE_WAVEFRONT));
}
__device__ __forceinline__ void lds_st8(v2f *p, v2f v)
{
    __hip_atomic_store(reinterpret_cast<unsigned long long *>(p), __builtin_bit_cast(unsigned long long, v),
                       __ATOMIC_RELAXED, __HIP_MEMORY_SCOPE_WAVEFRONT);
}


__host__ __device__ __forceinline__ int lds_pad(int pos) { return pos + ((pos >> 5) << 1); }

}
```

cutesdr_amd/csrc/host_math.hpp:

```cpp
#pragma once
#include <cmath>
#include <complex>
#include <map>
#include <memory>
#include <mutex>
#include <vector>
#include "ref_constants.hpp"

namespace csdr {

typedef std::complex<double> cd;
constexpr double kTwoPi = 2.0 * 3.14159265358979323846;
constexpr double kPi = 3.14159265358979323846;

inline std::shared_ptr<const std::vector<double>> host_twiddles(size_t n)
{
    static std::mutex m;
    static std::map<size_t, std::shared_ptr<const std::vector<double>>> cache;
    std::lock_guard<std::mutex> g(m);
    auto it = cache.find(n);
    if (it != cache.end()) return it->second;
    auto t = std::make_shared<std::vector<double>>(n);
    for (size_t j = 0; j < n / 2; j++) {
        const double ang = kTwoPi * (double)j / (double)n;
        (*t)[2 * j] = std::cos(ang); (*t)[2 * j + 1] = std::sin(ang);
    }
    cache[n] = t;
    return t;
}
inline std::vector<double> design_twiddles(size_t n)
{
    std::vector<double> t(n);
    const long double two_pi = 2.0L * 3.14159265358979323846264338327950288L;
    for (size_t j = 0; j < n / 2; j++) {
        const long double ang = two_pi * (long double)j / (long double)n;
        t[2 * j] = (double)cosl(ang); t[2 * j + 1] = (double)sinl(ang);
    }
    return t;
}
inline std::shared_ptr<const std::vector<double>> fastfir_window(int p)
{
    static std::mutex m;
    static std::map<int, std::shared_ptr<const std::vector<double>>> cache;
    std::lock_guard<std::mutex> g(m);
    auto it = cache.find(p);
    if (it != cache.end()) return it->second;
    auto w = std::make_shared<std::vector<double>>(p);
    for (int i = 0; i < p; i++)
        (*w)[i] = refc::FF_WIN_A0 - refc::FF_WIN_A1 * std::cos((kTwoPi * i) / (p - 1)) +
                  refc::FF_WIN_A2 * std::cos((2.0 * kTwoPi * i) / (p - 1)) -
                  refc::FF_WIN_A3 * std::cos((3.0 * kTwoPi * i) / (p - 1));
    cache[p] = w;
    return w;
}

inline void host_fft(std::vector<cd> &a, int sign)
{
    const size_t n = a.size();
    const auto tw = host_twiddles(n);
    const double *T = tw->data();
    for (size_t i = 1, j = 0; i < n; i++) {
        size_t bit = n >> 1;
        for (; j & bit; bit >>= 1) j ^= bit;
        j ^= bit;
        if (i < j) std::swap(a[i], a[j]);
    }
    for (size_t len = 2; len <= n; len <<= 1) {
        const size_t half = len >> 1;
        for (size_t k = 0; k < half; k++) {
            const size_t j = k * (n / len);
            const cd w(T[2 * j], sign >= 0 ? T[2 * j + 1] : -T[2 * j + 1]);
            for (size_t b = k; b < n; b += len) {
                const cd u = a[b], v = a[b + half] * w;
                a[b] = u + v;
                a[b + half] = u - v;
            }
        }
    }
}

inline bool fastfir_design_job(double flo, double fhi, double offset, double fs, double &nfc, double &nfs)
{
    flo += offset;
    fhi += offset;
    if (flo >= fhi || flo >= fs / 2.0 || flo <= -fs / 2.0 || fhi >= fs / 2.0 || fhi <= -fs / 2.0)
        return false;
    const double nfl = flo / fs, nfh = fhi / fs;
    nfc = (nfh - nfl) / 2.0;
    nfs = kTwoPi * (nfh + nfl) / 2.0;
    return true;
}

inline bool fastfir_design(int n, double flo, double fhi, double offset, double fs, std::vector<cd> &H)
{
    const int p = n / 2 + 1;
    double nfc, nfs;
    if (!fastfir_design_job(flo, fhi, offset, fs, nfc, nfs)) return false;
    const double centre = 0.5 * (double)(p - 1);
    H.assign(n, cd(0.0, 0.0));
    const auto win = fastfir_window(p);
    for (int i = 0; i < p; i++) {
        const double x = (double)i - centre;
        double z;
        if ((double)i == centre) {
            z = 2.0 * nfc;
        } else {
            const double w = (*win)[i];
            z = std::sin(kTwoPi * x * nfc) / (kPi * x) * w;
        }
        H[i] = cd(z * std::cos(nfs * x) / (double)n, z * std::sin(nfs * x) / (double)n);
    }
    host_fft(H, +1);
    return true;
}

}
```

Before: 204,900 MSamples/s.

## Use real per-bin gain with quarter-block shift in 16K FastFIR kernel

For N=16384 with a self-designed filter, the kernel now multiplies the spectrum by a real gain per bin folded into the first inverse butterfly (bfly_gain), in place of a full complex filter multiply. It applies a quarter-block output shift so the inverse pass needs only a middle-tail butterfly. Gains come from the design kernel and host upload under a new permutation, and an optional register-resident twiddle path is added. This halves the filter coefficient bytes per bin and drops arithmetic in the multiply and last stage, at the cost of more code paths and a fallback kernel for shared or non-own designs.

```diff
diff --git a/cutesdr_amd/csrc/capi_fastfir.hip b/cutesdr_amd/csrc/capi_fastfir.hip
--- a/cutesdr_amd/csrc/capi_fastfir.hip
+++ b/cutesdr_amd/csrc/capi_fastfir.hip
@@ -26,6 +26,8 @@
     bool per_channel;
     float *d_h;
     float *d_h2;
+    float *d_gain;
+    bool own_design;
     float *d_hist;
     int hist_cur;
     int dbg_stage; float *dbg_out;
@@ -34,12 +36,13 @@
     double flo, fhi, off, fs;
     std::vector<std::vector<cd>> resp;
     std::vector<int> perm, perm2;
+    std::vector<int> permg;
     PatchQueue patches;
     std::vector<DesignJob> jobs;
     std::vector<int> job_of;
     std::vector<char> stale;
     double *d_win = nullptr, *d_tw = nullptr;
-    int *d_perm = nullptr, *d_perm2 = nullptr;
+    int *d_perm = nullptr, *d_perm2 = nullptr, *d_permg = nullptr;
     double *d_resp = nullptr;
     hipEvent_t ev_design = nullptr;
 };
@@ -73,7 +76,7 @@
     if (!rc) {
         DesignArgs a;
         a.jobs = (const DesignJob *)d; a.win = b->d_win; a.tw = b->d_tw; a.perm = b->d_perm; a.perm2 = b->d_perm2;
-        a.h = b->d_h; a.h2 = b->d_h2; a.resp = b->d_resp;
+        a.h = b->d_h; a.h2 = b->d_h2; a.resp = b->d_resp; a.permg = b->d_permg; a.gain = b->d_gain;
         e = fastfir_design_launch(b->log2n, a, (int)b->jobs.size(), s);
         if (e == hipSuccess) {
             for (const DesignJob &j : b->jobs) b->job_of[j.slot] = -1;
@@ -109,10 +112,12 @@
     if (!b->d_tw) CSDR_HIP(hipMalloc((void **)&b->d_tw, n * sizeof(double)));
     if (!b->d_perm) CSDR_HIP(hipMalloc((void **)&b->d_perm, n * sizeof(int)));
     if (!b->d_perm2) CSDR_HIP(hipMalloc((void **)&b->d_perm2, n * sizeof(int)));
+    if (!b->d_permg) CSDR_HIP(hipMalloc((void **)&b->d_permg, n * sizeof(int)));
     CSDR_HIP(hipMemcpy(b->d_win, win->data(), p * sizeof(double), hipMemcpyHostToDevice));
     CSDR_HIP(hipMemcpy(b->d_tw, tw.data(), n * sizeof(double), hipMemcpyHostToDevice));
     CSDR_HIP(hipMemcpy(b->d_perm, b->perm.data(), n * sizeof(int), hipMemcpyHostToDevice));
     CSDR_HIP(hipMemcpy(b->d_perm2, b->perm2.data(), n * sizeof(int), hipMemcpyHostToDevice));
+    CSDR_HIP(hipMemcpy(b->d_permg, b->permg.data(), n * sizeof(int), hipMemcpyHostToDevice));
     CSDR_HIP(hipMalloc((void **)&b->d_resp, (size_t)b->channels * n * sizeof(cd)));
     return CSDR_OK;
 }
@@ -132,6 +137,10 @@
             for (int t = 0; t < T; t++)
                 for (int e = 0; e < 2; e++) b->perm2[(j * T + t) * 2 + e] = fastfir2_bin_of(b->log2n, t, j, e);
     }
+    b->permg.resize(b->n);
+    for (int i = 0; i < 8; i++)
+        for (int t = 0; t < T; t++)
+            for (int c = 0; c < 4; c++) b->permg[(i * T + t) * 4 + c] = fastfir2_gain_bin_of(b->log2n, t, i, c);
 }
 
 static int upload_response(csdr_fastfir_batch *b, int slot, const std::vector<cd> &H)
@@ -149,7 +158,8 @@
         const int rc = b->patches.add(dst + (size_t)slot * 2 * b->n, dev.data(), dev.size() * sizeof(float));
         if (rc) return rc;
     }
-    return CSDR_OK;
+    for (int i = 0; i < b->n; i++) dev[i] = (float)fastfir_gain(H[b->permg[i]], b->permg[i]);
+    return b->patches.add(b->d_gain + (size_t)slot * b->n, dev.data(), (size_t)b->n * sizeof(float));
 }
 
 static int set_response(csdr_fastfir_batch *b, int slot, const std::vector<cd> &H)
@@ -185,7 +195,8 @@
         const char *v = getenv("CSDR_FASTFIR_VARIANT");
         b->variant = (v && atoi(v) == 0) ? 0 : 2;
     }
-    b->d_h = b->d_h2 = b->d_hist = b->d_tw1 = b->d_tw2 = nullptr;
+    b->d_h = b->d_h2 = b->d_gain = b->d_hist = b->d_tw1 = b->d_tw2 = nullptr;
+    b->own_design = true;
     b->flo = -1.0; b->fhi = 1.0; b->off = 1.0; b->fs = 1.0;
     build_perm(b);
     const size_t hbytes = (size_t)fft_size * 8, histbytes = 2 * (size_t)channels * (fft_size / 2) * 8;
@@ -201,6 +212,7 @@
         }
     bool ok = hipMalloc((void **)&b->d_h, hbytes) == hipSuccess &&
               hipMalloc((void **)&b->d_h2, hbytes) == hipSuccess && hipMemset(b->d_h2, 0, hbytes) == hipSuccess &&
+              hipMalloc((void **)&b->d_gain, hbytes / 2) == hipSuccess && hipMemset(b->d_gain, 0, hbytes / 2) == hipSuccess &&
               hipMalloc((void **)&b->d_hist, histbytes) == hipSuccess &&
               hipMalloc((void **)&b->d_tw1, 8192) == hipSuccess &&
               hipMalloc((void **)&b->d_tw2, 8192) == hipSuccess &&
@@ -225,6 +237,7 @@
     (void)hipSetDevice(b->device);
     if (b->d_h) (void)hipFree(b->d_h);
     if (b->d_h2) (void)hipFree(b->d_h2);
+    if (b->d_gain) (void)hipFree(b->d_gain);
     if (b->d_hist) (void)hipFree(b->d_hist);
     if (b->d_tw1) (void)hipFree(b->d_tw1);
     if (b->d_tw2) (void)hipFree(b->d_tw2);
@@ -233,6 +246,7 @@
     if (b->d_tw) (void)hipFree(b->d_tw);
     if (b->d_perm) (void)hipFree(b->d_perm);
     if (b->d_perm2) (void)hipFree(b->d_perm2);
+    if (b->d_permg) (void)hipFree(b->d_permg);
     if (b->d_resp) (void)hipFree(b->d_resp);
     delete b;
 }
@@ -268,6 +282,14 @@
             CSDR_HIP(hipFree(b->d_h2));
             b->d_h2 = nh2;
         }
+        {
+            float *ng = nullptr;
+            CSDR_HIP(hipMalloc((void **)&ng, one / 2 * b->channels));
+            for (int c = 0; c < b->channels; c++)
+                CSDR_HIP(hipMemcpy((char *)ng + one / 2 * c, b->d_gain, one / 2, hipMemcpyDeviceToDevice));
+            CSDR_HIP(hipFree(b->d_gain));
+            b->d_gain = ng;
+        }
         b->resp.resize(b->channels, b->resp[0]);
         b->per_channel = true;
     }
@@ -359,6 +381,7 @@
     a.hist = (const v2f_h *)(b->d_hist + b->hist_cur * hist_half);
     a.hist_next = (v2f_h *)(b->d_hist + (b->hist_cur ^ 1) * hist_half);
     a.h = (const v4f_h *)b->d_h; a.tw1 = (const v2f_h *)b->d_tw1; a.tw2 = (const v2f_h *)b->d_tw2;
+    a.gain = nullptr;
     a.in_stride = in_stride; a.out_stride = out_stride;
     a.h_stride = b->per_channel ? b->n / 2 : 0;
     a.channels = b->channels;
@@ -381,6 +404,7 @@
     a.dbg_stage = b->dbg_stage; a.dbg = (v2f_h *)b->dbg_out;
     if (b->variant >= 2) {
         a.h = (const v4f_h *)b->d_h2;
+        if (b->log2n == 14 && b->own_design) a.gain = (const v4f_h *)b->d_gain;
         CSDR_HIP(fastfir2_launch(b->log2n, a, s));
     }
     else CSDR_HIP(fastfir_launch(b->log2n, a, s));
@@ -405,6 +429,7 @@
     const int slot = dst->per_channel ? dr : 0;
     int rc = set_response(dst, slot, H);
     if (rc) return rc;
+    dst->own_design = dst->own_design && src->own_design;
     dst->flo = dst->fhi = dst->off = dst->fs = std::nan("");
     return CSDR_OK;
 }
diff --git a/cutesdr_amd/csrc/capi_hosttest.hip b/cutesdr_amd/csrc/capi_hosttest.hip
--- a/cutesdr_amd/csrc/capi_hosttest.hip
+++ b/cutesdr_amd/csrc/capi_hosttest.hip
@@ -6,9 +6,27 @@
 #include "testgen_host.hpp"
 #include "scope_host.hpp"
 #include "fastfir_kernels.h"
+#include "fft_core.hpp"
 #include <cstring>
 
 using namespace csdr;
+
+template <int SIGN> static void host_head4_gain(const float *x4, const float *g4, float *out4)
+{
+    v2f x[4];
+    for (int q = 0; q < 4; q++) x[q] = v2f{x4[2 * q], x4[2 * q + 1]};
+    dit_head4_gain<0, 4, SIGN>(x, v2f{g4[0], g4[1]}, v2f{g4[2], g4[3]});
+    for (int q = 0; q < 4; q++) { out4[2 * q] = x[q].x; out4[2 * q + 1] = x[q].y; }
+}
+template <int R, int SIGN> static void host_dft_middle(const float *in, float *out)
+{
+    v2f x[R];
+    for (int n = 0; n < R; n++) x[bitrev<R>(n)] = v2f{in[2 * n], in[2 * n + 1]};
+    static_for<0, R / 4>([&](auto G) { dit_head4<G.value, R, SIGN>(x); });
+    if constexpr (R == 32) dit_single<8, 32, SIGN>(x);
+    static_for<0, R / 4>([&](auto I) { dit_tail_middle<I.value, R, SIGN>(x); });
+    for (int r = 0; r < R / 2; r++) { out[2 * r] = x[R / 4 + r].x; out[2 * r + 1] = x[R / 4 + r].y; }
+}
 
 extern "C" {
 
@@ -24,6 +42,30 @@
     return fastfir_design_job(flo, fhi, off, fs, *nfc, *nfs) ? 0 : -1;
 }
 int csdr__host_fastfir_bin_of(int log2n, int t, int r) { return fastfir_bin_of(log2n, t, r); }
+int csdr__host_fastfir_gains(int n, double flo, double fhi, double off, double fs, double *h_out, double *p_out)
+{
+    std::vector<cd> H;
+    if (!fastfir_design(n, flo, fhi, off, fs, H)) return -1;
+    memcpy(h_out, H.data(), sizeof(cd) * n);
+    for (int k = 0; k < n; k++) p_out[k] = fastfir_gain(H[k], k);
+    return 0;
+}
+int csdr__host_fastfir2_bin_of(int log2n, int t, int j, int e) { return fastfir2_bin_of(log2n, t, j, e); }
+int csdr__host_fastfir2_gain_bin_of(int log2n, int t, int i, int c) { return fastfir2_gain_bin_of(log2n, t, i, c); }
+
+void csdr__host_dit_head4_gain(int sign, const float *x4, const float *g4, float *out4)
+{
+    if (sign > 0) host_head4_gain<+1>(x4, g4, out4); else host_head4_gain<-1>(x4, g4, out4);
+}
+int csdr__host_dft_middle(int r, int sign, const float *in, float *out)
+{
+    if (r == 16 && sign > 0) host_dft_middle<16, +1>(in, out);
+    else if (r == 16) host_dft_middle<16, -1>(in, out);
+    else if (r == 32 && sign > 0) host_dft_middle<32, +1>(in, out);
+    else if (r == 32) host_dft_middle<32, -1>(in, out);
+    else return -1;
+    return 0;
+}
 
 int csdr__host_dc_plan(double in_rate, double bw, int *codes, double *out_rate, int *warmup)
 {
diff --git a/cutesdr_amd/csrc/fastfir2_kernels.hip b/cutesdr_amd/csrc/fastfir2_kernels.hip
--- a/cutesdr_amd/csrc/fastfir2_kernels.hip
+++ b/cutesdr_amd/csrc/fastfir2_kernels.hip
@@ -16,6 +16,12 @@
 #endif
 #ifndef K1_HREG
 #define K1_HREG 8
+#endif
+#ifndef K1_REALGAIN
+#define K1_REALGAIN 1
+#endif
+#ifndef K1_TWREG
+#define K1_TWREG 0
 #endif
 #ifndef K1_HREG4K
 #define K1_HREG4K 4
@@ -56,16 +62,17 @@
     static constexpr int LDS_BYTES = (VW * Base::LDS_DATA + 1024) * 8;
 };
 
-template <int LOG2N>
-__global__ __launch_bounds__(K1Cfg<LOG2N>::T) __attribute__((amdgpu_waves_per_eu(2, 2)))
-void fastfir_os2_kernel(FastFirArgs a)
+template <int LOG2N, bool RG>
+__device__ __forceinline__ void fastfir_os2_body(const FastFirArgs a)
 {
     CSDR_WG_TRACE_SCOPE(a.trace, WGT_FF);
+    static_assert(!RG || LOG2N == 14, "the quarter-block shift is whole rows of the outer pass at N = 16384 only");
     using Cfg = FastFirCfg<LOG2N>;
     constexpr int N = Cfg::N, T = Cfg::T, R0 = Cfg::R0, G = Cfg::G, L = N / 2;
     constexpr int HALF = R0 / 2;
     constexpr int VW = K1Cfg<LOG2N>::VW;
-    constexpr int HREG = LOG2N == 12 ? K1_HREG4K : (LOG2N == 11 ? K1_HREG2K : K1_HREG);
+    constexpr int HREG = RG ? 0 : (LOG2N == 12 ? K1_HREG4K : (LOG2N == 11 ? K1_HREG2K : K1_HREG));
+    constexpr int TWREG = RG ? K1_TWREG : 0;
     static_assert(R0 == 16 || R0 == 8 || R0 == 4 || R0 == 2, "the grouped outer pass is written for N = 2048 ... 16384");
     auto block_barrier = [] {
         if constexpr (LOG2N == 11) {
@@ -107,6 +114,7 @@
     const rsrc_t r_hist = make_rsrc(a.hist + (long)ch * L, L * 8u);
     const rsrc_t r_out = make_rsrc(a.out + (long)ch * a.out_stride, (unsigned)a.nblocks * L * 8u);
     const rsrc_t r_h = make_rsrc(a.h + (long)ch * a.h_stride, N * 8u);
+    const rsrc_t r_g = make_rsrc(a.gain + (long)ch * (a.h_stride / 2), N * 4u);
     constexpr int PSTEP = 2 * T, PSTEP_LDS = PSTEP + 2 * (PSTEP / 32), PSTEP_B = PSTEP * 8;
     const int voff = t * 16;
     auto load_half = [&](rsrc_t r, int soff, v2f (&dst)[16]) {
@@ -136,9 +144,14 @@
         for (int e = 0; e < G; e++) twiddle_powers<R0>(opaque(w1[e]), pw[e]);
     }
 
-    v4f hv[16];
+    v4f hv[RG ? 1 : 16];
 #pragma unroll
     for (int j = 0; j < HREG; j++) hv[j] = buf_load16(r_h, t * 16, j * (T * 16));
+    v4f pv[RG ? 8 : 1];
+    if constexpr (RG) {
+#pragma unroll
+        for (int i = 0; i < 8; i++) pv[i] = buf_load16(r_g, t * 16, i * (T * 16));
+    }
 #ifdef K1_ABLATE
     v4f habl = {1.0f, 0.0f, 1.0f, 0.0f};
     asm volatile("" : "+v"(habl));
@@ -155,6 +168,14 @@
     const int sb = t >> 5, sn = t & 31;
     v2f *const col = lds + lds_pad(1024 * sb) + sn;
     const v2f *const twc = tw2 + sn;
+    v2f twr[TWREG > 0 ? TWREG : 1];
+#pragma unroll
+    for (int k1 = 1; k1 <= TWREG; k1++) twr[k1 - 1] = a.tw2[32 * k1 + sn];
+    auto pass_tw = [&](auto K1) {
+        constexpr int k1 = K1.value;
+        if constexpr (k1 <= TWREG) return twr[k1 - 1];
+        else return lds_ld8(twc + 32 * k1);
+    };
     v2f *const rowp = lds + 34 * t;
     v2f *const outer = lds + lds_pad(2 * t);
     constexpr int OUTER_ROW = 1024 + 2 * (1024 / 32);
@@ -303,7 +324,7 @@
 #ifdef ABL_TW
             static_for<1, 4>([&](auto P) { tw[0][P.value] = twabl; });
 #else
-            static_for<1, 4>([&](auto P) { tw[0][P.value] = lds_ld8(twc + 32 * (8 * P.value)); });
+            static_for<1, 4>([&](auto P) { tw[0][P.value] = pass_tw(std::integral_constant<int, 8 * P.value>{}); });
 #endif
             CSDR_SB();
             CSDR_STAMP(8);
@@ -313,14 +334,14 @@
 #ifdef ABL_TW
                     static_for<0, 4>([&](auto P) { tw[(i + 1) & 1][P.value] = twabl; });
 #else
-                    static_for<0, 4>([&](auto P) { tw[(i + 1) & 1][P.value] = lds_ld8(twc + 32 * (i + 1 + 8 * P.value)); });
+                    static_for<0, 4>([&](auto P) { tw[(i + 1) & 1][P.value] = pass_tw(std::integral_constant<int, i + 1 + 8 * P.value>{}); });
 #endif
                 if constexpr (i < 8) {
 #ifdef ABL_H
-                    hv[2 * i] = habl; hv[2 * i + 1] = habl;
-#else
-                    if constexpr (2 * i >= HREG) hv[2 * i] = buf_load16(r_h, t * 16, (2 * i) * (T * 16));
-                    if constexpr (2 * i + 1 >= HREG) hv[2 * i + 1] = buf_load16(r_h, t * 16, (2 * i + 1) * (T * 16));
+                    if constexpr (!RG) { hv[2 * i] = habl; hv[2 * i + 1] = habl; }
+#else
+                    if constexpr (!RG && 2 * i >= HREG) hv[2 * i] = buf_load16(r_h, t * 16, (2 * i) * (T * 16));
+                    if constexpr (!RG && 2 * i + 1 >= HREG) hv[2 * i + 1] = buf_load16(r_h, t * 16, (2 * i + 1) * (T * 16));
 #endif
                     dit_tail<i, 32, +1>(x);
                     static_for<0, 4>([&](auto P) {
@@ -364,8 +385,11 @@
                 constexpr int i = Ii.value, g = bitrev<8>(i);
                 dit_tail<i, 32, +1>(x);
                 y[4 * g] = x[i]; y[4 * g + 1] = x[i + 16]; y[4 * g + 2] = x[i + 8]; y[4 * g + 3] = x[i + 24];
-                dit_head4_tw<g, 32, -1>(y, v2f{hv[2 * i].x, hv[2 * i].y}, v2f{hv[2 * i].z, hv[2 * i].w},
-                                        v2f{hv[2 * i + 1].x, hv[2 * i + 1].y}, v2f{hv[2 * i + 1].z, hv[2 * i + 1].w});
+                if constexpr (RG)
+                    dit_head4_gain<g, 32, -1>(y, v2f{pv[i].x, pv[i].y}, v2f{pv[i].z, pv[i].w});
+                else
+                    dit_head4_tw<g, 32, -1>(y, v2f{hv[2 * i].x, hv[2 * i].y}, v2f{hv[2 * i].z, hv[2 * i].w},
+                                            v2f{hv[2 * i + 1].x, hv[2 * i + 1].y}, v2f{hv[2 * i + 1].z, hv[2 * i + 1].w});
                 if constexpr ((i & 1) == 1) CSDR_SB();
             });
 #pragma unroll
@@ -414,7 +438,7 @@
 #ifdef ABL_TW
                     if constexpr (r != 0) tw[r] = twabl;
 #else
-                    if constexpr (r != 0) tw[r] = lds_ld8(twc + 32 * bitrev<32>(r));
+                    if constexpr (r != 0) tw[r] = pass_tw(std::integral_constant<int, bitrev<32>(r)>{});
 #endif
                 });
             };
@@ -479,10 +503,17 @@
                 static_for<0, R0 / 4 + 1>([&](auto I) {
                     constexpr int i = I.value;
                     if constexpr (i < R0 / 4) {
-                        dit_tail_upper<i, R0, -1>(y[0]);
-                        dit_tail_upper<i, R0, -1>(y[1]);
-                        sv[2 * i] = store_operand(y[0][i + 8], y[1][i + 8]);
-                        sv[2 * i + 1] = store_operand(y[0][i + 12], y[1][i + 12]);
+                        if constexpr (RG) {
+                            dit_tail_middle<i, R0, -1>(y[0]);
+                            dit_tail_middle<i, R0, -1>(y[1]);
+                            sv[2 * i] = store_operand(y[0][i + 4], y[1][i + 4]);
+                            sv[2 * i + 1] = store_operand(y[0][i + 8], y[1][i + 8]);
+                        } else {
+                            dit_tail_upper<i, R0, -1>(y[0]);
+                            dit_tail_upper<i, R0, -1>(y[1]);
+                            sv[2 * i] = store_operand(y[0][i + 8], y[1][i + 8]);
+                            sv[2 * i + 1] = store_operand(y[0][i + 12], y[1][i + 12]);
+                        }
                     }
                     if constexpr (i > 0) {
                         CSDR_STORE_GROUP_BEGIN();
@@ -588,20 +619,33 @@
 }
 
 template <int LOG2N>
+__global__ __launch_bounds__(K1Cfg<LOG2N>::T) __attribute__((amdgpu_waves_per_eu(2, 2)))
+void fastfir_os2_kernel(FastFirArgs a)
+{
+    fastfir_os2_body<LOG2N, LOG2N == 14 && K1_REALGAIN>(a);
+}
+__global__ __launch_bounds__(K1Cfg<14>::T) __attribute__((amdgpu_waves_per_eu(2, 2)))
+void fastfir_os2h_kernel(FastFirArgs a)
+{
+    fastfir_os2_body<14, false>(a);
+}
+
+template <int LOG2N>
 static hipError_t launch2_one(const FastFirArgs &a, hipStream_t stream)
 {
     using Cfg = K1Cfg<LOG2N>;
-    hipError_t e = CSDR_MAX_LDS_ONCE(&fastfir_os2_kernel<LOG2N>, Cfg::LDS_BYTES);
+    void (*kernel)(FastFirArgs) = &fastfir_os2_kernel<LOG2N>;
+    if (LOG2N == 14 && !(K1_REALGAIN && a.gain)) kernel = &fastfir_os2h_kernel;
+    hipError_t e = kernel == &fastfir_os2h_kernel ? CSDR_MAX_LDS_ONCE(&fastfir_os2h_kernel, Cfg::LDS_BYTES)
+                                                  : CSDR_MAX_LDS_ONCE(&fastfir_os2_kernel<LOG2N>, Cfg::LDS_BYTES);
     if (e != hipSuccess) return e;
 #ifdef CSDR_WG_TRACE
     FastFirArgs b = a;
     b.trace = wgtrace_next();
-    hipLaunchKernelGGL((fastfir_os2_kernel<LOG2N>), dim3((a.channels * a.runs + Cfg::VW - 1) / Cfg::VW), dim3(Cfg::T),
-                       Cfg::LDS_BYTES, stream, b);
+    hipLaunchKernelGGL(kernel, dim3((a.channels * a.runs + Cfg::VW - 1) / Cfg::VW), dim3(Cfg::T), Cfg::LDS_BYTES, stream, b);
     return hipGetLastError();
 #endif
-    hipLaunchKernelGGL((fastfir_os2_kernel<LOG2N>), dim3((a.channels * a.runs + Cfg::VW - 1) / Cfg::VW), dim3(Cfg::T),
-                       Cfg::LDS_BYTES, stream, a);
+    hipLaunchKernelGGL(kernel, dim3((a.channels * a.runs + Cfg::VW - 1) / Cfg::VW), dim3(Cfg::T), Cfg::LDS_BYTES, stream, a);
     return hipGetLastError();
 }
 
@@ -623,5 +667,9 @@
     const int k2 = i + 8 * h + 16 * e;
     return (t >> 5) + R0 * ((t & 31) + 32 * k2);
 }
-
-}
+int fastfir2_gain_bin_of(int log2n, int t, int i, int c)
+{
+    return fastfir2_bin_of(log2n, t, 2 * i + (c >> 1), c & 1);
+}
+
+}
diff --git a/cutesdr_amd/csrc/fastfir_design_kernels.h b/cutesdr_amd/csrc/fastfir_design_kernels.h
--- a/cutesdr_amd/csrc/fastfir_design_kernels.h
+++ b/cutesdr_amd/csrc/fastfir_design_kernels.h
@@ -15,6 +15,8 @@
     const double *tw;
     const int *perm, *perm2;
     float *h, *h2;
+    const int *permg;
+    float *gain;
     double *resp;
 };
 
diff --git a/cutesdr_amd/csrc/fastfir_design_kernels.hip b/cutesdr_amd/csrc/fastfir_design_kernels.hip
--- a/cutesdr_amd/csrc/fastfir_design_kernels.hip
+++ b/cutesdr_amd/csrc/fastfir_design_kernels.hip
@@ -67,11 +67,16 @@
 
     v2f_d *h = reinterpret_cast<v2f_d *>(a.h) + (size_t)job.slot * N;
     v2f_d *h2 = reinterpret_cast<v2f_d *>(a.h2) + (size_t)job.slot * N;
+    float *gain = a.gain + (size_t)job.slot * N;
     for (int i = tid; i < N; i += T) {
         const v2d p = w[a.perm[i]], p2 = w[a.perm2[i]];
         v2f_d f = {(float)p.x, (float)p.y}, f2 = {(float)p2.x, (float)p2.y};
         h[i] = f;
         h2[i] = f2;
+        const int kg = a.permg[i];
+        const v2d pg = w[kg];
+        const double gr = (kg & 1) ? pg.y : pg.x;
+        gain[i] = (float)((kg & 2) ? -gr : gr);
         if constexpr (Cfg::IN_LDS) row[i] = w[i];
     }
 }
diff --git a/cutesdr_amd/csrc/fastfir_kernels.h b/cutesdr_amd/csrc/fastfir_kernels.h
--- a/cutesdr_amd/csrc/fastfir_kernels.h
+++ b/cutesdr_amd/csrc/fastfir_kernels.h
@@ -13,6 +13,7 @@
     v2f_h *hist_next;
     v2f_h *out;
     const v4f_h *h;
+    const v4f_h *gain;
     const v2f_h *tw1;
     const v2f_h *tw2;
     long in_stride;
@@ -34,5 +35,6 @@
 
 hipError_t fastfir2_launch(int log2n, const FastFirArgs &a, hipStream_t stream);
 int fastfir2_bin_of(int log2n, int t, int j, int e);
+int fastfir2_gain_bin_of(int log2n, int t, int i, int c);
 
 }
diff --git a/cutesdr_amd/csrc/fft_core.hpp b/cutesdr_amd/csrc/fft_core.hpp
--- a/cutesdr_amd/csrc/fft_core.hpp
+++ b/cutesdr_amd/csrc/fft_core.hpp
@@ -309,6 +309,44 @@
     bfly_dit<0, SIGN>(x[a], x[a + 2]);
     bfly_dit<8, SIGN>(x[a + 1], x[a + 3]);
 }
+__host__ __device__ __forceinline__ void bfly_gain(v2f &xa, v2f &xb, v2f g)
+{
+#if CSDR_PK_ASM
+    v2f t, a, b;
+    asm("v_pk_mul_f32 %0, %1, %2 op_sel:[0,0] op_sel_hi:[1,0]" : "=v"(t) : "v"(xa), "v"(g));
+    asm("v_pk_fma_f32 %0, %1, %2, %3 op_sel:[0,1,0] op_sel_hi:[1,1,1]" : "=v"(a) : "v"(xb), "v"(g), "v"(t));
+    asm("v_pk_fma_f32 %0, %1, %2, %3 op_sel:[0,1,0] op_sel_hi:[1,1,1] neg_lo:[0,1,0] neg_hi:[0,1,0]"
+        : "=v"(b) : "v"(xb), "v"(g), "v"(t));
+    xa = a; xb = b;
+#else
+    const v2f t = xa * g.xx, v = xb * g.yy;
+    xa = t + v; xb = t - v;
+#endif
+}
+template <int G, int R, int SIGN>
+__host__ __device__ __forceinline__ void dit_head4_gain(v2f (&x)[R], v2f g01, v2f g23)
+{
+    constexpr int a = 4 * G;
+    bfly_gain(x[a], x[a + 1], g01);
+    bfly_gain(x[a + 2], x[a + 3], g23);
+    bfly_dit<0, SIGN>(x[a], x[a + 2]);
+    bfly_dit<8, SIGN>(x[a + 1], x[a + 3]);
+}
+template <int K, int SIGN>
+__host__ __device__ __forceinline__ void bfly_dit_sum(v2f &xa, const v2f xb)
+{
+    if constexpr (K == 0) {
+        xa = xa + xb;
+    } else if constexpr (K == 8) {
+        xa = add_jv<SIGN>(xa, xb);
+    } else {
+        constexpr float c = kCos32[K];
+        constexpr float s = (SIGN > 0 ? 1.0f : -1.0f) * kCos32[(K + 24) & 31];
+        const v2f w1 = {c, s}, w2 = {-s, c};
+        const v2f t = __builtin_elementwise_fma(xb.xx, w1, xa);
+        xa = __builtin_elementwise_fma(xb.yy, w2, t);
+    }
+}
 template <int K, int SIGN>
 __host__ __device__ __forceinline__ void bfly_dit_lower(const v2f xa, v2f &xb)
 {
@@ -335,6 +373,16 @@
     bfly_dit_lower<(I + Q) * (32 / R), SIGN>(x[I + Q], x[I + 3 * Q]);
 }
 template <int I, int R, int SIGN>
+__host__ __device__ __forceinline__ void dit_tail_middle(v2f (&x)[R])
+{
+    static_assert(R >= 8 && I < R / 4, "dit_tail_middle");
+    constexpr int Q = R / 4;
+    bfly_dit<I *(64 / R), SIGN>(x[I], x[I + Q]);
+    bfly_dit<I *(64 / R), SIGN>(x[I + 2 * Q], x[I + 3 * Q]);
+    bfly_dit_lower<I *(32 / R), SIGN>(x[I], x[I + 2 * Q]);
+    bfly_dit_sum<(I + Q) * (32 / R), SIGN>(x[I + Q], x[I + 3 * Q]);
+}
+template <int I, int R, int SIGN>
 __host__ __device__ __forceinline__ void dit_tail(v2f (&x)[R])
 {
     static_assert(R >= 8 && I < R / 4, "dit_tail");
diff --git a/cutesdr_amd/csrc/host_math.hpp b/cutesdr_amd/csrc/host_math.hpp
--- a/cutesdr_amd/csrc/host_math.hpp
+++ b/cutesdr_amd/csrc/host_math.hpp
@@ -114,4 +114,14 @@
     return true;
 }
 
+inline double fastfir_gain(const cd &h, int k)
+{
+    switch (k & 3) {
+    case 0: return h.real();
+    case 1: return h.imag();
+    case 2: return -h.real();
+    default: return -h.imag();
+    }
 }
+
+}
```

After: 211,500 MSamples/s (median of 6 runs). +3.2%, better.
